# fujii-team/Henbun

Measured on AMD Instinct MI355X. Metric: elbo_samples_per_sec, higher is better.
Workload: dtype f32; 1 GPU; cfg2 SVGP ELBO step: 1-D UnitRBF, N=1e6, M=512 inducing, minibatch 8192 per GPU, diag Normal q(u), diagonal residual, Adam lr 1e-3; global_batch=8192, per_gpu_batch=8192, parallelism=dp1, N=1000000, M=512, dp_exchange=none, dp_ranks=1, contraction=native, tri_pack=False

## Files before the change

henbun_amd/csrc/chain.cuh:

```cuda
#ifndef HB_CHAIN_CUH
#define HB_CHAIN_CUH
#include "common.cuh"
#include "ew_prog.cuh"

enum { HB_CHAIN_PROG = 1, HB_CHAIN_ADAM = 2, HB_CHAIN_GLL = 3, HB_CHAIN_SGP_FINISH = 4, HB_CHAIN_GRAM_ELL = 5, HB_CHAIN_GLL_FOLD = 6 };
#define HB_CHAIN_MAX_JOBS 6
#define HB_CHAIN_PROG_MAX_N 4096
#define HB_CHAIN_FINISH_MAX_N 512
#define HB_CHAIN_GLL_MAX_N 4096
#define HB_CHAIN_ADAM_MAX_N 4096
#define HB_CHAIN_ELL_MAX_N 16384
#define HB_CHAIN_GLL_FOLD_MAX_N 4096

enum { HB_CHAIN_READ = 1, HB_CHAIN_WRITE = 2, HB_CHAIN_RW = 3 };

struct HbChainJob {
  int kind = 0, is64 = 0;
  const void* p[HB_PROG_MAX_IN + HB_PROG_MAX_OUT] = {};
  long l[8] = {};
  double d[8] = {};
  ProgArgs prog;
  int reduces = 0;
  long ext[HB_PROG_MAX_IN + HB_PROG_MAX_OUT] = {};
  unsigned char role[HB_PROG_MAX_IN + HB_PROG_MAX_OUT] = {};
  void span(int k, long bytes, int r) {
    ext[k] = p[k] != nullptr && bytes > 0 ? bytes : 0;
    role[k] = (unsigned char)r;
  }
};

bool hb_chain_recording();
int hb_chain_push(const HbChainJob& job, hipStream_t stream);
int hb_chain_flush(hipStream_t stream);

#endif
```

henbun_amd/csrc/chain_bodies.cuh:

```cuda
#ifndef HB_CHAIN_BODIES_CUH
#define HB_CHAIN_BODIES_CUH

#pragma clang fp contract(off)

__device__ __forceinline__ long hb_opaque_zero() {
  int z = 0;
  asm volatile("" : "+v"(z));
  return (long)z;
}

template <typename T>
struct HbAdamStatus {
  long tnow, fail0;
  T dpf;
  int w0;
};
template <typename T>
__device__ __forceinline__ void hb_adam_status_load(const long* t, const int* info, long n_info, const T* dpflag, const long* fail,
                                                    HbAdamStatus<T>& s) {
  const long z = hb_opaque_zero();
  const long* fp = fail != nullptr ? fail : t;
  const T* dp = dpflag != nullptr ? dpflag : reinterpret_cast<const T*>(t);
  const int* ip = n_info > 0 ? info + ((long)threadIdx.x < n_info ? (long)threadIdx.x : n_info - 1) : reinterpret_cast<const int*>(t);
  s.tnow = t[z];
// ... 263 lines not shown
  hb_gauss_fold_load<T, 1>(partial, nb, h);
  hb_gauss_fold_body<T, 1>(h, partial, nb, ll, dscale, dvar, smem, mir);
}

template <typename T>
__device__ __forceinline__ void sgp_finish_one(const T* __restrict__ part, int gy, long idx, T epsv, T* __restrict__ f,
                                               T* __restrict__ v, T* __restrict__ eps_out, long n, long P, int diagonal) {
  const long e = idx / n, j = idx - e * n;
  const T* pp = part + e * gy * 5 * n + j;
  T s = T(0);
  for (int y = 0; y < gy; ++y) s += pp[(long)y * 5 * n];
  const T vv = T(1) - s;
  v[idx] = vv;
  if (eps_out) eps_out[idx] = epsv;
  const T scale = diagonal ? hb_sqrt(hb_abs(vv)) * epsv : T(0);
  for (long p = 0; p < P; ++p) {
    T mean = T(0);
    for (int y = 0; y < gy; ++y) mean += pp[((long)y * 5 + 1 + p) * n];
    f[(e * P + p) * n + j] = mean + scale;
  }
}

template <typename T>
__device__ __forceinline__ void hb_sgp_finish_body(const T* __restrict__ part, int gy, const T* __restrict__ eps_in, uint64_t* rng,
                                                   long nlanes, T* __restrict__ eps_out, T* __restrict__ f, T* __restrict__ v,
                                                   long total, long n, long P, int diagonal, long t0, long nthreads) {
  const long npairs = (total + 1) / 2;
  if (rng) {
    const long nact = nlanes < npairs ? nlanes : npairs;
    for (long t = t0; t < nact; t += nthreads) {
      HbRng g = rng_load(rng, nlanes, t);
      for (long p = t; p < npairs; p += nlanes) {
        T z0, z1;
        g.normal2(z0, z1);
        sgp_finish_one<T>(part, gy, 2 * p, z0, f, v, eps_out, n, P, diagonal);
        if (2 * p + 1 < total) sgp_finish_one<T>(part, gy, 2 * p + 1, z1, f, v, eps_out, n, P, diagonal);
      }
      rng_store(rng, nlanes, t, g);
    }
  } else {
    for (long idx = t0; idx < total; idx += nthreads)
      sgp_finish_one<T>(part, gy, idx, eps_in ? eps_in[idx] : T(0), f, v, (eps_out != eps_in) ? eps_out : nullptr, n, P, diagonal);
  }
}

template <typename T, int D>
__device__ __forceinline__ void hb_gram_ell_load(const T* __restrict__ partial, long rows, long d, long dl, long c, T (&h)[D]) {
  const long cnt = dl == 1 ? rows * d : rows;
#pragma unroll
  for (int k = 0; k < D; ++k) {
    const long t = (long)threadIdx.x + (long)k * blockDim.x, tc = t < cnt ? t : cnt - 1;
    h[k] = dl == 1 ? partial[tc] : partial[tc * d + c];
  }
}
template <typename T, int D>
__device__ __forceinline__ void hb_gram_ell_body(const T (&h)[D], const T* __restrict__ partial, long rows, long d, long dl, long c,
                                                 T* __restrict__ ellbar, T* smem, T* mir = nullptr) {
  const long cnt = dl == 1 ? rows * d : rows;
  T acc = T(0);
#pragma unroll
  for (int k = 0; k < D; ++k)
    if ((long)threadIdx.x + (long)k * blockDim.x < cnt) acc += h[k];
  if (dl == 1) {
#pragma unroll 4
    for (long t = (long)threadIdx.x + (long)D * blockDim.x; t < cnt; t += blockDim.x) acc += partial[t];
  } else {
#pragma unroll 4
    for (long r = (long)threadIdx.x + (long)D * blockDim.x; r < cnt; r += blockDim.x) acc += partial[r * d + c];
  }
  acc = block_sum(acc, smem);
  if (threadIdx.x == 0) {
    ellbar[c] = acc;
    if (mir) mir[0] = acc;
  }
}
template <typename T>
__device__ __forceinline__ void hb_gram_ell_body(const T* __restrict__ partial, long rows, long d, long dl, long c,
                                                 T* __restrict__ ellbar, T* smem, T* mir = nullptr) {
  T h[1];
  hb_gram_ell_load<T, 1>(partial, rows, d, dl, c, h);
  hb_gram_ell_body<T, 1>(h, partial, rows, d, dl, c, ellbar, smem, mir);
}

template <typename T, int D>
__device__ __forceinline__ void hb_chain_win_load(const T* base, long n, T (&h)[D]) {
#pragma unroll
  for (int k = 0; k < D; ++k) {
    const long i = (long)threadIdx.x + (long)k * blockDim.x;
    h[k] = base[i < n ? i : hb_opaque_zero()];
  }
}
template <typename T, int D>
__device__ __forceinline__ void hb_chain_win_store(T* win, long n, const T (&h)[D]) {
#pragma unroll
  for (int k = 0; k < D; ++k) {
    const long i = (long)threadIdx.x + (long)k * blockDim.x;
    if (i < n) win[i] = h[k];
  }
}
template <typename T>
__device__ __forceinline__ void hb_chain_mirror(const T* p, T v, const T* base, long n, T* win) {
  const long ob = (long)p - (long)base;
  if (ob >= 0 && ob < n * (long)sizeof(T)) win[ob / (long)sizeof(T)] = v;
}
__device__ __forceinline__ void hb_chain_sync() { __syncthreads(); }

#pragma clang fp contract(fast)
#endif
```

henbun_amd/csrc/gram.hip:

```cpp
#include "common.cuh"
#include "../../include/henbun_hip.h"
#include "chain.cuh"
#include "gram_value.cuh"

template <typename T>
__global__ void __launch_bounds__(256) gram_fwd_kernel(int kind, const T* __restrict__ X, long sX,
                                                       const T* __restrict__ X2, long sX2, const T* __restrict__ ell,
                                                       long sEll, long dl, T* __restrict__ K, long B, long n, long n2,
                                                       long d, T diag_add) {
  const long total = B * n * n2;
  const long stride = (long)gridDim.x * blockDim.x;
  for (long t = (long)blockIdx.x * blockDim.x + threadIdx.x; t < total; t += stride) {
    const long b = t / (n * n2);
    const long rem = t - b * n * n2;
    const long i = rem / n2, j = rem - i * n2;
    const T kv = gram_value<T>(kind, X + b * sX + i * d, X2 + b * sX2 + j * d, ell + b * sEll, dl, d);
    K[t] = (i == j) ? kv + diag_add : kv;
  }
}

template <typename T>
static int gram_fwd(int kind, const T* X, long sX, const T* X2, long sX2, const T* ell, long sEll, long dl, T* K,
                    long B, long n, long n2, long d, double diag_add, hipStream_t stream) {
  HB_REQUIRE(kind >= HB_KERN_RBF && kind <= HB_KERN_SQDIST, "hb_gram_fwd: unknown kernel kind %d", kind);
// ... 95 lines not shown
template <typename T>
static int gram_bwd(int kind_flags, const T* X, long sX, const T* X2, long sX2, const T* ell, long sEll, long dl,
                    const T* Kbar, T* Xbar, T* X2bar, T* ellbar, long B, long n, long n2, long d, T* ws,
                    hipStream_t stream) {
  const int kind = kind_flags & ~HB_KERN_KBAR_SYMMETRIC;
  HB_REQUIRE(kind >= HB_KERN_RBF && kind <= HB_KERN_SQDIST, "hb_gram_bwd: unknown kernel kind %d", kind);
  HB_REQUIRE(B >= 0 && n >= 0 && n2 >= 0 && d >= 1, "hb_gram_bwd: bad extents");
  HB_REQUIRE(dl == 1 || dl == d, "hb_gram_bwd: lengthscales must have 1 or d entries");
  HB_REQUIRE(sEll == 0 || sEll == dl, "hb_gram_bwd: lengthscale batch stride must be 0 or dl");
  HB_REQUIRE(X && X2 && ell && Kbar, "hb_gram_bwd: NULL pointer");
  HB_REQUIRE(!ellbar || ws, "hb_gram_bwd: ellbar needs workspace");
  HB_REQUIRE(B <= 65535, "hb_gram_bwd: batch too large");
  if (B == 0) return 0;
  if (hb_chain_recording()) {
    const int crc = hb_chain_flush(stream);
    if (crc) return crc;
  }
  if (n == 0 || n2 == 0) {
    if (Xbar && n > 0) HB_HIP(hb_zero_async(Xbar, sizeof(T) * B * n * d, stream));
    if (X2bar && n2 > 0) HB_HIP(hb_zero_async(X2bar, sizeof(T) * B * n2 * d, stream));
    if (ellbar) HB_HIP(hb_zero_async(ellbar, sizeof(T) * dl * (sEll != 0 ? B : 1), stream));
    return 0;
  }
  const bool sym = Xbar && X2bar == Xbar;
  const bool kbar_sym = (kind_flags & HB_KERN_KBAR_SYMMETRIC) != 0;
  HB_REQUIRE(!kbar_sym || sym, "hb_gram_bwd: HB_KERN_KBAR_SYMMETRIC only applies to the one-pass form (X2 == X, X2bar == Xbar)");
  HB_REQUIRE(!sym || (X == X2 && sX == sX2 && n == n2), "hb_gram_bwd: Xbar == X2bar requires X2 == X");
  if (Xbar || ellbar) {
    hipLaunchKernelGGL(gram_bwd_side_kernel<T>, dim3(n, B), dim3(256), 0, stream, kind, sym ? (kbar_sym ? 3 : 2) : 0, X, sX, X2, sX2, ell, sEll,
                       dl, Kbar, Xbar, ellbar ? ws : (T*)nullptr, n, n2, d);
    HB_LAUNCH_CHECK();
    if (ellbar) {
      const long rows_ = sEll != 0 ? n : B * n, groups_ = sEll != 0 ? B : 1;
      if (hb_chain_recording() && rows_ * d * groups_ <= HB_CHAIN_ELL_MAX_N && groups_ * dl <= 16 && !(X2bar && !sym)) {
        HbChainJob j;
        j.kind = HB_CHAIN_GRAM_ELL;
        j.is64 = sizeof(T) == 8;
        j.p[0] = ws, j.p[1] = ellbar;
        j.l[0] = rows_, j.l[1] = d, j.l[2] = dl, j.l[3] = groups_;
        j.span(0, groups_ * rows_ * d * (long)sizeof(T), HB_CHAIN_READ), j.span(1, groups_ * dl * (long)sizeof(T), HB_CHAIN_WRITE);
        return hb_chain_push(j, stream);
      }
      if (sEll != 0)
        hipLaunchKernelGGL(gram_ell_finish_kernel<T>, dim3(dl, B), dim3(256), 0, stream, ws, n, d, dl, ellbar);
      else
        hipLaunchKernelGGL(gram_ell_finish_kernel<T>, dim3(dl, 1), dim3(256), 0, stream, ws, B * n, d, dl, ellbar);
      HB_LAUNCH_CHECK();
    }
  }
  if (X2bar && !sym) {
    hipLaunchKernelGGL(gram_bwd_side_kernel<T>, dim3(n2, B), dim3(256), 0, stream, kind, 1, X, sX, X2, sX2, ell, sEll,
                       dl, Kbar, X2bar, (T*)nullptr, n, n2, d);
    HB_LAUNCH_CHECK();
  }
  return 0;
}
template <typename T>
static int gram_ell_fold(const T* partial, long rows, long d, long dl, long groups, T* ellbar, hipStream_t stream) {
  HB_REQUIRE(partial && ellbar && rows >= 1 && d >= 1 && groups >= 1 && (dl == 1 || dl == d), "hb_gram_ell_fold: bad arguments");
  if (hb_chain_recording() && rows * d * groups <= HB_CHAIN_ELL_MAX_N && groups * dl <= 16) {
    HbChainJob j;
    j.kind = HB_CHAIN_GRAM_ELL;
    j.is64 = sizeof(T) == 8;
    j.p[0] = partial, j.p[1] = ellbar;
    j.l[0] = rows, j.l[1] = d, j.l[2] = dl, j.l[3] = groups;
    j.span(0, groups * rows * d * (long)sizeof(T), HB_CHAIN_READ), j.span(1, groups * dl * (long)sizeof(T), HB_CHAIN_WRITE);
    return hb_chain_push(j, stream);
  }
  if (hb_chain_recording()) {
    const int crc = hb_chain_flush(stream);
    if (crc) return crc;
  }
  hipLaunchKernelGGL(gram_ell_finish_kernel<T>, dim3(dl, groups), dim3(256), 0, stream, partial, rows, d, dl, ellbar);
  HB_LAUNCH_CHECK();
  return 0;
}
extern "C" int hb_gram_ell_fold_f32(const float* partial, long rows, long d, long dl, long groups, float* ellbar, void* stream) {
  return gram_ell_fold<float>(partial, rows, d, dl, groups, ellbar, (hipStream_t)stream);
}
extern "C" int hb_gram_ell_fold_f64(const double* partial, long rows, long d, long dl, long groups, double* ellbar, void* stream) {
  return gram_ell_fold<double>(partial, rows, d, dl, groups, ellbar, (hipStream_t)stream);
}

extern "C" int hb_gram_bwd_f32(int kind, const float* X, long sX, const float* X2, long sX2, const float* ell,
                               long sEll, long dl, const float* Kbar, float* Xbar, float* X2bar, float* ellbar,
                               long B, long n, long n2, long d, float* ws, void* stream) {
  return gram_bwd<float>(kind, X, sX, X2, sX2, ell, sEll, dl, Kbar, Xbar, X2bar, ellbar, B, n, n2, d, ws,
                         (hipStream_t)stream);
}
extern "C" int hb_gram_bwd_f64(int kind, const double* X, long sX, const double* X2, long sX2, const double* ell,
                               long sEll, long dl, const double* Kbar, double* Xbar, double* X2bar, double* ellbar,
                               long B, long n, long n2, long d, double* ws, void* stream) {
  return gram_bwd<double>(kind, X, sX, X2, sX2, ell, sEll, dl, Kbar, Xbar, X2bar, ellbar, B, n, n2, d, ws,
                          (hipStream_t)stream);
}
```

henbun_amd/csrc/jit.hip:

```cpp
#include "common.cuh"
#include "../../include/henbun_hip.h"
#include "ew_prog.cuh"
#include "chain.cuh"
#include <dlfcn.h>
#include <stdarg.h>
#include <stdio.h>
#include <string.h>
#include <hip/hiprtc.h>
#include <map>
#include <mutex>
#include <string>
#include <vector>
#include "_gen/ew_jit_prelude.inc"

namespace {

struct Rtc {
  bool ok = false;
  hiprtcResult (*create)(hiprtcProgram*, const char*, const char*, int, const char**, const char**) = nullptr;
  hiprtcResult (*compile)(hiprtcProgram, int, const char**) = nullptr;
  hiprtcResult (*log_size)(hiprtcProgram, size_t*) = nullptr;
  hiprtcResult (*log)(hiprtcProgram, char*) = nullptr;
  hiprtcResult (*code_size)(hiprtcProgram, size_t*) = nullptr;
  hiprtcResult (*code)(hiprtcProgram, char*) = nullptr;
// ... 368 lines not shown
            height[r] > 1 ? "q" : "0");
  }
  s += "  }\n}\n";
  if (source_out && source_cap > 0) snprintf(source_out, (size_t)source_cap, "%s", s.c_str() + (sizeof(HB_EW_JIT_PRELUDE) - 1));
  if (!handle_out) {
    std::vector<char> co;
    return compile_to_code(s, &co);
  }
  Compiled c;
  const int rc = compile_source(s, &c);
  if (rc) return rc;
  JitProgram* p = new JitProgram;
  p->colprog = true;
  p->is64 = sizeof(T) == 8;
  p->fn = c.fn;
  p->n = n;
  p->grid = (unsigned)hb_stream_grid(n, 256);
  for (int k = 0; k < nin; ++k) p->ptrs.push_back(const_cast<void*>(in[k]));
  for (int k = 0; k < nout; ++k) p->ptrs.push_back(out[k]);
  for (size_t k = 0; k < p->ptrs.size(); ++k) p->argv.push_back(&p->ptrs[k]);
  *handle_out = p;
  return 0;
}

}

extern "C" int hb_ewise_colprog_build_f32(int ninstr, const int* code, const double* params, int nin, const void* const* in,
                                          const long* istrides, int nout, void* const* out, const int* out_regs,
                                          const long* ostrides, long R, long n, void** handle_out, char* source_out,
                                          long source_cap) {
  return colprog_build<float>(ninstr, code, params, nin, in, istrides, nout, out, out_regs, ostrides, R, n, handle_out, source_out,
                              source_cap);
}
extern "C" int hb_ewise_colprog_build_f64(int ninstr, const int* code, const double* params, int nin, const void* const* in,
                                          const long* istrides, int nout, void* const* out, const int* out_regs,
                                          const long* ostrides, long R, long n, void** handle_out, char* source_out,
                                          long source_cap) {
  return colprog_build<double>(ninstr, code, params, nin, in, istrides, nout, out, out_regs, ostrides, R, n, handle_out, source_out,
                               source_cap);
}

extern "C" int hb_ewise_jit_available(void) { return rtc().ok ? 1 : 0; }

extern "C" int hb_ewise_jit_build_f32(int ninstr, const int* code, const double* params, int nin, const void* const* in,
                                      const long* istrides, int nout, void* const* out, const int* out_regs,
                                      const long* ostrides, int ndim, const long* shape, void** handle_out, long* n_out,
                                      int* reduces_out, char* source_out, long source_cap) {
  return jit_build<float>(ninstr, code, params, nin, in, istrides, nout, out, out_regs, ostrides, ndim, shape, handle_out,
                          n_out, reduces_out, source_out, source_cap);
}
extern "C" int hb_ewise_jit_build_f64(int ninstr, const int* code, const double* params, int nin, const void* const* in,
                                      const long* istrides, int nout, void* const* out, const int* out_regs,
                                      const long* ostrides, int ndim, const long* shape, void** handle_out, long* n_out,
                                      int* reduces_out, char* source_out, long source_cap) {
  return jit_build<double>(ninstr, code, params, nin, in, istrides, nout, out, out_regs, ostrides, ndim, shape, handle_out,
                           n_out, reduces_out, source_out, source_cap);
}

namespace {

struct ChainState {
  bool recording = false;
  std::vector<HbChainJob> jobs;
};
thread_local ChainState g_chain;

struct HbChainArgs {
  const void* p[64];
  long l[48];
  double d[16];
};

constexpr int CHAIN_NSTAMP = 16;
unsigned long long* g_chain_stamps = nullptr;
const void* chain_stamp_buffer() { return g_chain_stamps; }
static void chain_job_slots(const HbChainJob& j, int* p, int* l, int* d) {
  switch (j.kind) {
    case HB_CHAIN_PROG: *p = j.prog.nin + j.prog.nout, *l = 0, *d = 0; break;
    case HB_CHAIN_ADAM: *p = 8, *l = 3, *d = 5; break;
    case HB_CHAIN_GLL: *p = 9, *l = 1, *d = 1; break;
    case HB_CHAIN_GLL_FOLD: *p = 4, *l = 1, *d = 0; break;
    case HB_CHAIN_SGP_FINISH: *p = 6, *l = 6, *d = 0; break;
    case HB_CHAIN_GRAM_ELL: *p = 2, *l = 4, *d = 0; break;
    default: *p = 20, *l = 8, *d = 8; break;
  }
}

int chain_source_plain(const std::vector<HbChainJob>& jobs, std::string* out, HbChainArgs* args, int* np_out, int* nl_out, int* nd_out,
                       bool stamps) {
  const bool is64 = jobs[0].is64 != 0;
  std::string s;
  int np = 0, nl = 0, nd = 0;
  auto P = [&](const void* v) { HbChainArgs& a = *args; a.p[np] = v; return np++; };
  auto L = [&](long v) { HbChainArgs& a = *args; a.l[nl] = v; return nl++; };
  auto D = [&](double v) { HbChainArgs& a = *args; a.d[nd] = v; return nd++; };
  for (size_t q = 0; q < jobs.size(); ++q) {
    const HbChainJob& j = jobs[q];
    HB_REQUIRE((j.is64 != 0) == is64, "hb_chain: jobs of different element types in one chain");
    HB_REQUIRE(np + 20 <= 64 && nl + 8 <= 48 && nd + 8 <= 16, "hb_chain: argument block exhausted");
    if (q) s += "  __syncthreads();\n";
    s += "  {\n";
    if (j.kind == HB_CHAIN_PROG) {
      const ProgArgs& G = j.prog;
      for (int k = 0; k < G.nin; ++k) appendf(s, "  const T* in%d = (const T*)A.p[%d];\n", k, P(j.p[k]));
      for (int k = 0; k < G.nout; ++k) appendf(s, "  T* out%d = (T*)A.p[%d];\n", k, P(j.p[G.nin + k]));
      char loop[96];
      snprintf(loop, sizeof(loop), "for (long i = threadIdx.x; i < %ldL; i += 1024) {", G.n);
      emit_program(s, G, loop);
    } else if (j.kind == HB_CHAIN_ADAM) {
      const int p0 = P(j.p[0]); P(j.p[1]); P(j.p[2]); P(j.p[3]); P(j.p[4]); P(j.p[5]); P(j.p[6]); P(j.p[7]);
      const int l0 = L(j.l[0]); L(j.l[1]); L(j.l[2]);
      const int d0 = D(j.d[0]); D(j.d[1]); D(j.d[2]); D(j.d[3]); D(j.d[4]);
      appendf(s, "  hb_adam_body<T>((T*)A.p[%d], (const T*)A.p[%d], (T*)A.p[%d], (T*)A.p[%d], A.l[%d], A.d[%d], A.d[%d], A.d[%d], "
                 "A.d[%d], A.d[%d], (long*)A.p[%d], (int)A.l[%d], (const int*)A.p[%d], A.l[%d], (const T*)A.p[%d], (long*)A.p[%d], "
                 "(long)threadIdx.x, 1024L, true, true);\n",
              p0, p0 + 1, p0 + 2, p0 + 3, l0, d0, d0 + 1, d0 + 2, d0 + 3, d0 + 4, p0 + 4, l0 + 2, p0 + 5, l0 + 1, p0 + 6, p0 + 7);
    } else if (j.kind == HB_CHAIN_GLL) {
      const int p0 = P(j.p[0]); P(j.p[1]); P(j.p[2]); P(j.p[3]); P(j.p[4]); P(j.p[5]); P(j.p[6]); P(j.p[7]); P(j.p[8]);
      const int l0 = L(j.l[0]);
      const int d0 = D(j.d[0]);
      appendf(s, "  hb_gauss_ll_single_body<T>((const T*)A.p[%d], (const T*)A.p[%d], (const T*)A.p[%d], (const T*)A.p[%d], A.l[%d], "
                 "(T*)A.p[%d], (T*)A.p[%d], (T*)A.p[%d], (T*)A.p[%d], smem, (T*)A.p[%d], (T)A.d[%d]);\n",
              p0, p0 + 1, p0 + 2, p0 + 3, l0, p0 + 4, p0 + 5, p0 + 6, p0 + 7, p0 + 8, d0);
    } else if (j.kind == HB_CHAIN_GLL_FOLD) {
      const int p0 = P(j.p[0]); P(j.p[1]); P(j.p[2]); P(j.p[3]);
      const int l0 = L(j.l[0]);
      appendf(s, "  hb_gauss_fold_body<T>((const T*)A.p[%d], A.l[%d], (T*)A.p[%d], (T*)A.p[%d], (T*)A.p[%d], smem);\n", p0, l0, p0 + 1,
              p0 + 2, p0 + 3);
    } else if (j.kind == HB_CHAIN_SGP_FINISH) {
      const int p0 = P(j.p[0]); P(j.p[1]); P(j.p[2]); P(j.p[3]); P(j.p[4]); P(j.p[5]);
      const int l0 = L(j.l[0]); L(j.l[1]); L(j.l[2]); L(j.l[3]); L(j.l[4]); L(j.l[5]);
      appendf(s, "  hb_sgp_finish_body<T>((const T*)A.p[%d], (int)A.l[%d], (const T*)A.p[%d], (uint64_t*)A.p[%d], A.l[%d], (T*)A.p[%d], "
                 "(T*)A.p[%d], (T*)A.p[%d], A.l[%d], A.l[%d], A.l[%d], (int)A.l[%d], (long)threadIdx.x, 1024L);\n",
              p0, l0, p0 + 1, p0 + 2, l0 + 1, p0 + 3, p0 + 4, p0 + 5, l0 + 2, l0 + 3, l0 + 4, l0 + 5);
    } else if (j.kind == HB_CHAIN_GRAM_ELL) {
      const int p0 = P(j.p[0]); P(j.p[1]);
      const int l0 = L(j.l[0]); L(j.l[1]); L(j.l[2]); L(j.l[3]);
      appendf(s, "  for (long grp = 0; grp < A.l[%d]; ++grp)\n    for (long c = 0; c < A.l[%d]; ++c)\n"
                 "      hb_gram_ell_body<T>((const T*)A.p[%d] + grp * A.l[%d] * A.l[%d], A.l[%d], A.l[%d], A.l[%d], c, "
                 "(T*)A.p[%d] + grp * A.l[%d], smem);\n",
              l0 + 3, l0 + 2, p0, l0, l0 + 1, l0, l0 + 1, l0 + 2, p0 + 1, l0 + 2);
    } else {
      HB_REQUIRE(false, "hb_chain: unknown job kind %d", j.kind);
    }
    s += "  }\n";
    if (stamps) appendf(s, "  const unsigned long long hb_st%d = clock64();\n", (int)q + 2);
  }
  if (stamps) {
    HB_REQUIRE(np < 64, "hb_chain: no pointer slot left for the stamps");
    const int ps = P(chain_stamp_buffer());
    appendf(s, "  if (threadIdx.x == 0) {\n    unsigned long long* sb = (unsigned long long*)A.p[%d];\n    sb[0] = %dULL; sb[1] = hb_st0; sb[2] = hb_st0;\n", ps,
            (int)jobs.size() + 2);
    for (size_t q = 0; q < jobs.size(); ++q) appendf(s, "    sb[%d] = hb_st%d;\n", (int)q + 3, (int)q + 2);
    s += "  }\n";
  }
  s += "}\n";
  std::string h = HB_EW_JIT_PRELUDE;
  h += "\n#define HB_JIT_OPAQUE(x) asm volatile(\"\" : \"+v\"(x))";
  appendf(h, "\nstruct HbChainArgs { const void* p[%d]; long l[%d]; double d[%d]; };", np > 0 ? np : 1, nl > 0 ? nl : 1, nd > 0 ? nd : 1);
  appendf(h, "\ntypedef %s T;\nextern \"C\" __global__ void __launch_bounds__(1024) hb_jit_kernel(const HbChainArgs Ain) {\n",
          is64 ? "double" : "float");
  h += "  __shared__ T smem[16];\n  const HbChainArgs A = Ain;\n";
  if (stamps) h += "  const unsigned long long hb_st0 = clock64();\n";
  *out = h + s;
  *np_out = np, *nl_out = nl, *nd_out = nd;
  return 0;
}

enum { CH_PLAIN = 0, CH_EXT = 1, CH_SLOT = 2, CH_WIN = 3 };
constexpr long CHAIN_WIN_BYTES = 40960;
constexpr int CHAIN_MAX_WIN = 8, CHAIN_MAX_SLOT = 16;
constexpr int CHAIN_HOIST_REGS = 40;

struct ChainWin {
  int job, idx;
  int cap;
  std::string nexpr;
};
struct ChainMirror { int kind, id; };
struct ChainCls { int kind = CH_PLAIN, id = -1; };

struct ChainPlan {
  const std::vector<HbChainJob>& jobs;
  size_t esz;
  std::vector<int> pbase, lbase, dbase;
  std::vector<ChainWin> wins;
  int nslot = 0;
  long win_bytes = 0;
  std::vector<std::vector<std::vector<ChainMirror>>> mirrors;
  std::vector<std::vector<int>> slot_of;

  explicit ChainPlan(const std::vector<HbChainJob>& j) : jobs(j), esz(j[0].is64 ? 8 : 4) {
    int np = 0, nl = 0, nd = 0;
    for (const HbChainJob& q : jobs) {
      pbase.push_back(np), lbase.push_back(nl), dbase.push_back(nd);
      int a, b, c;
      chain_job_slots(q, &a, &b, &c);
      np += a, nl += b, nd += c;
    }
    mirrors.assign(jobs.size(), std::vector<std::vector<ChainMirror>>(HB_PROG_MAX_IN + HB_PROG_MAX_OUT));
    slot_of.assign(jobs.size(), std::vector<int>(HB_PROG_MAX_IN + HB_PROG_MAX_OUT, -1));
  }
  static bool overlap(const HbChainJob& a, int i, const HbChainJob& b, int k) {
    const char *a0 = (const char*)a.p[i], *b0 = (const char*)b.p[k];
    return a.ext[i] > 0 && b.ext[k] > 0 && a0 < b0 + b.ext[k] && b0 < a0 + a.ext[i];
  }
  int capability(int j, int k) const {
    const HbChainJob& J = jobs[j];
    switch (J.kind) {
      case HB_CHAIN_PROG: return k >= J.prog.nin ? 2 : 0;
      case HB_CHAIN_ADAM: return k == 0 ? 2 : 0;
      case HB_CHAIN_GLL: return k >= 5 && k <= 7 ? 1 : 0;
      case HB_CHAIN_GLL_FOLD: return k >= 1 && k <= 3 ? 1 : 0;
      case HB_CHAIN_GRAM_ELL: return k == 1 && J.ext[1] == (long)esz ? 1 : 0;
      default: return 0;
    }
  }
  int slot(int j, int k) {
    if (slot_of[j][k] >= 0) return slot_of[j][k];
    const int kind = jobs[j].kind;
    const bool triple = kind == HB_CHAIN_GLL || kind == HB_CHAIN_GLL_FOLD;
    const int first = kind == HB_CHAIN_GLL ? 5 : kind == HB_CHAIN_GLL_FOLD ? 1 : k, count = triple ? 3 : 1;
    if (nslot + count > CHAIN_MAX_SLOT) return -1;
    for (int c = 0; c < count; ++c) slot_of[j][first + c] = nslot + c;
    nslot += count;
    return slot_of[j][k];
  }
  bool external(int q, int k) const {
    for (int j = 0; j < q; ++j)
      for (int o = 0; o < HB_PROG_MAX_IN + HB_PROG_MAX_OUT; ++o)
        if ((jobs[j].role[o] & HB_CHAIN_WRITE) && overlap(jobs[q], k, jobs[j], o)) return false;
    return true;
  }
  ChainCls classify(int q, int k, long n, const std::string& nexpr) {
    ChainCls c;
    const HbChainJob& Q = jobs[q];
    if (Q.ext[k] <= 0) return c;
    std::vector<std::pair<int, int>> prod;
    for (int j = 0; j < q; ++j)
      for (int o = 0; o < HB_PROG_MAX_IN + HB_PROG_MAX_OUT; ++o)
        if ((jobs[j].role[o] & HB_CHAIN_WRITE) && overlap(Q, k, jobs[j], o)) prod.push_back({j, o});
    if (prod.empty()) {
      c.kind = CH_EXT;
      return c;
    }
    if (prod.size() == 1 && n == 1) {
      const int j = prod[0].first, o = prod[0].second;
      if (jobs[j].p[o] == Q.p[k] && jobs[j].ext[o] == (long)esz && capability(j, o) >= 1) {
        const int sl = slot(j, o);
        if (sl < 0) return c;
        mirrors[j][o].push_back({CH_SLOT, sl});
        c.kind = CH_SLOT, c.id = sl;
        return c;
      }
    }
    int cap = 1;
    while (cap < n) cap *= 2;
    if ((int)wins.size() >= CHAIN_MAX_WIN || n < 1 || win_bytes + (long)cap * (long)esz > CHAIN_WIN_BYTES) return c;
    for (const auto& jo : prod) {
      const long off = (const char*)jobs[jo.first].p[jo.second] - (const char*)Q.p[k];
      if (capability(jo.first, jo.second) != 2 || off % (long)esz != 0) return c;
    }
    const int w = (int)wins.size();
    wins.push_back({q, k, cap, nexpr});
    win_bytes += (long)cap * (long)esz;
    for (const auto& jo : prod) mirrors[jo.first][jo.second].push_back({CH_WIN, w});
    c.kind = CH_WIN, c.id = w;
    return c;
  }
  std::string mirror_text(int j, int k) const {
    std::string t;
    for (const ChainMirror& m : mirrors[j][k]) {
      if (m.kind == CH_SLOT) {
        appendf(t, "hb_slot[%d] = %%V; ", m.id);
      } else {
        const ChainWin& W = wins[m.id];
        appendf(t, "hb_chain_mirror<T>(%%P, %%V, (const T*)A.p[%d], %s, hb_win%d); ", pbase[W.job] + W.idx, W.nexpr.c_str(), m.id);
      }
    }
    return t;
  }
  std::string mir_arg(int j, int k) const {
    char b[48];
    if (slot_of[j][k] >= 0)
      snprintf(b, sizeof(b), "hb_slot + %d", slot_of[j][k]);
    else
      snprintf(b, sizeof(b), "(T*)nullptr");
    return b;
  }
};

int chain_source_hoist(const std::vector<HbChainJob>& jobs, std::string* out, HbChainArgs* args, int* np_out, int* nl_out, int* nd_out,
                       bool stamps) {
  const bool is64 = jobs[0].is64 != 0;
  const int NQ = (int)jobs.size();
  int np = 0, nl = 0, nd = 0;
  auto P = [&](const void* v) { HbChainArgs& a = *args; a.p[np] = v; return np++; };
  auto L = [&](long v) { HbChainArgs& a = *args; a.l[nl] = v; return nl++; };
  auto D = [&](double v) { HbChainArgs& a = *args; a.d[nd] = v; return nd++; };
  ChainPlan plan(jobs);
  struct JobCls {
    ChainCls in[HB_PROG_MAX_IN];
    bool hoist = false;
    ChainCls g;
    bool tmv_ext = false, st_ext = false, part_ext = false;
    int depth = 1;
  };
  std::vector<JobCls> cls(NQ);
  for (int q = 0; q < NQ; ++q) {
    const HbChainJob& j = jobs[q];
    HB_REQUIRE((j.is64 != 0) == is64, "hb_chain: jobs of different element types in one chain");
    JobCls& c = cls[q];
    if (j.kind == HB_CHAIN_PROG) {
      const ProgArgs& G = j.prog;
      c.hoist = G.n >= 1 && G.n <= 1024;
      for (int k = 0; k < G.nin && c.hoist; ++k) {
        long n = 1;
        for (int d = 0; d < G.ndim; ++d) n += G.istr[k][d] * (long)(G.shape[d] - 1);
        char b[32];
        snprintf(b, sizeof(b), "%ldL", n);
        c.in[k] = plan.classify(q, k, n, b);
      }
    } else if (j.kind == HB_CHAIN_ADAM) {
      c.depth = (int)((j.l[0] + 1023) / 1024);
      c.tmv_ext = plan.external(q, 0) && plan.external(q, 2) && plan.external(q, 3);
      c.st_ext = plan.external(q, 4) && plan.external(q, 5) && plan.external(q, 6) && plan.external(q, 7);
      char b[32];
      snprintf(b, sizeof(b), "A.l[%d]", plan.lbase[q]);
      c.g = plan.classify(q, 1, j.l[0], b);
    } else if (j.kind == HB_CHAIN_GLL_FOLD) {
      c.part_ext = plan.external(q, 0);
      c.depth = (int)((j.l[0] + 1023) / 1024);
    } else if (j.kind == HB_CHAIN_GRAM_ELL) {
      c.part_ext = plan.external(q, 0);
      c.depth = (int)(((j.l[2] == 1 ? j.l[0] * j.l[1] : j.l[0]) + 1023) / 1024);
    }
    if (c.depth < 1) c.depth = 1;
  }
  int held = 0;
  for (const ChainWin& W : plan.wins) held += (W.cap > 1024 ? W.cap / 1024 : 1) * (is64 ? 2 : 1);
  auto fits = [&](int values) {
    const int regs = values * (is64 ? 2 : 1);
    if (held + regs > CHAIN_HOIST_REGS) return false;
    held += regs;
    return true;
  };
  for (int pass = 0; pass < 2; ++pass) {
    for (int q = 0; q < NQ; ++q) {
      const HbChainJob& j = jobs[q];
      JobCls& c = cls[q];
      if ((j.kind == HB_CHAIN_ADAM) != (pass == 0)) continue;
      if (j.kind == HB_CHAIN_ADAM) {
        if (c.tmv_ext && !fits(3 * c.depth)) c.tmv_ext = false;
        if (c.g.kind == CH_EXT && !fits(c.depth)) c.g.kind = CH_PLAIN;
      } else if (j.kind == HB_CHAIN_GLL_FOLD) {
        if (c.part_ext && !fits(3 * c.depth)) c.part_ext = false;
      } else if (j.kind == HB_CHAIN_GRAM_ELL) {
        if (c.part_ext && !fits(c.depth)) c.part_ext = false;
      } else if (j.kind == HB_CHAIN_PROG) {
        for (int k = 0; k < j.prog.nin; ++k)
          if (c.in[k].kind == CH_EXT && !fits(1)) c.in[k].kind = CH_PLAIN;
      }
    }
  }
  std::string top, s;
  for (size_t w = 0; w < plan.wins.size(); ++w) {
    const ChainWin& W = plan.wins[w];
    const int dw = W.cap > 1024 ? W.cap / 1024 : 1;
    appendf(top, "  T hb_wf%d[%d]; hb_chain_win_load<T, %d>((const T*)A.p[%d], %s, hb_wf%d);\n", (int)w, dw, dw, plan.pbase[W.job] + W.idx,
            W.nexpr.c_str(), (int)w);
  }
  for (int q = 0; q < NQ; ++q) {
    const HbChainJob& j = jobs[q];
    const JobCls& c = cls[q];
    HB_REQUIRE(np + 20 <= 64 && nl + 8 <= 48 && nd + 8 <= 16, "hb_chain: argument block exhausted");
    HB_REQUIRE(np == plan.pbase[q] && nl == plan.lbase[q] && nd == plan.dbase[q], "hb_chain: argument slots out of step");
    if (q) s += "  __syncthreads();\n";
    s += "  {\n";
    if (j.kind == HB_CHAIN_PROG) {
      const ProgArgs& G = j.prog;
      ProgHooks hooks;
      for (int k = 0; k < G.nin; ++k) appendf(s, "  const T* in%d = (const T*)A.p[%d];\n", k, P(j.p[k]));
      for (int k = 0; k < G.nout; ++k) appendf(s, "  T* out%d = (T*)A.p[%d];\n", k, P(j.p[G.nin + k]));
      bool any_ext = false;
      for (int k = 0; k < G.nin; ++k) any_ext = any_ext || c.in[k].kind == CH_EXT;
      if (any_ext) {
        appendf(top, "  const long h%di = (long)threadIdx.x < %ldL ? (long)threadIdx.x : 0L;\n  long h%drem = h%di;\n", q, G.n, q, q);
        for (int d = G.ndim - 1; d >= 0; --d) {
          if (d == 0)
            appendf(top, "  const long h%dx%d = h%drem;\n", q, d, q);
          else
            appendf(top, "  const long h%dx%d = h%drem %% %dL; h%drem /= %dL;\n", q, d, q, G.shape[d], q, G.shape[d]);
        }
      }
      for (int k = 0; k < G.nin; ++k) {
        char b[256];
        if (c.in[k].kind == CH_EXT) {
          bool uniform = true;
          for (int d = 0; d < G.ndim; ++d) uniform = uniform && G.istr[k][d] == 0;
          appendf(top, "  const T h%d_%d = ((const T*)A.p[%d])[%s", q, k, plan.pbase[q] + k, uniform ? "hb_opaque_zero()" : "0");
          for (int d = 0; d < G.ndim; ++d)
            if (G.istr[k][d] != 0) appendf(top, " + h%dx%d * %ldL", q, d, G.istr[k][d]);
          top += "];\n";
          snprintf(b, sizeof(b), "h%d_%d", q, k);
          hooks.in_expr[k] = b;
        } else if (c.in[k].kind == CH_SLOT) {
          snprintf(b, sizeof(b), "hb_slot[%d]", c.in[k].id);
          hooks.in_expr[k] = b;
        } else if (c.in[k].kind == CH_WIN) {
          std::string e;
          appendf(e, "hb_win%d[0", c.in[k].id);
          for (int d = 0; d < G.ndim; ++d)
            if (G.istr[k][d] != 0) appendf(e, " + x%d * %ldL", d, G.istr[k][d]);
          hooks.in_expr[k] = e + "]";
        }
      }
      for (int k = 0; k < G.nout; ++k) hooks.out_extra[k] = plan.mirror_text(q, G.nin + k);
      char loop[96];
      snprintf(loop, sizeof(loop), "for (long i = threadIdx.x; i < %ldL; i += 1024) {", G.n);
      emit_program(s, G, loop, &hooks);
    } else if (j.kind == HB_CHAIN_ADAM) {
      const int p0 = P(j.p[0]); P(j.p[1]); P(j.p[2]); P(j.p[3]); P(j.p[4]); P(j.p[5]); P(j.p[6]); P(j.p[7]);
      const int l0 = L(j.l[0]); L(j.l[1]); L(j.l[2]);
      const int d0 = D(j.d[0]); D(j.d[1]); D(j.d[2]); D(j.d[3]); D(j.d[4]);
      std::string status, tmv, lr, gload;
      appendf(top, "  HbAdamOps<T, %d> h%do; HbAdamStatus<T> h%ds;\n", c.depth, q, q);
      appendf(status, "  hb_adam_status_load<T>((const long*)A.p[%d], (const int*)A.p[%d], A.l[%d], (const T*)A.p[%d], (const long*)A.p[%d], h%ds);\n",
              p0 + 4, p0 + 5, l0 + 1, p0 + 6, p0 + 7, q);
      appendf(tmv, "  hb_adam_load_tmv<T, %d>((const T*)A.p[%d], (const T*)A.p[%d], (const T*)A.p[%d], A.l[%d], (long)threadIdx.x, 1024L, h%do);\n",
              c.depth, p0, p0 + 2, p0 + 3, l0, q);
      appendf(lr, "  const T h%dlr = hb_adam_lr<T>(A.d[%d], A.d[%d], A.d[%d], h%ds.tnow);\n", q, d0, d0 + 1, d0 + 2, q);
      if (c.g.kind == CH_WIN)
        appendf(gload, "  hb_adam_load_g<T, %d>(hb_win%d, A.l[%d], (long)threadIdx.x, 1024L, h%do);\n", c.depth, c.g.id, l0, q);
      else
        appendf(gload, "  hb_adam_load_g<T, %d>((const T*)A.p[%d], A.l[%d], (long)threadIdx.x, 1024L, h%do);\n", c.depth, p0 + 1, l0, q);
      (c.st_ext ? top : s) += status;
      (c.tmv_ext ? top : s) += tmv;
      (c.g.kind == CH_EXT ? top : s) += gload;
      const int lr_slot = c.st_ext && q > 0 && plan.nslot < CHAIN_MAX_SLOT ? plan.nslot++ : -1;
      if (lr_slot >= 0) {
        appendf(top, "  if ((threadIdx.x >> 6) == 15) {\n  %s    if ((threadIdx.x & 63) == 0) hb_slot[%d] = h%dlr;\n  }\n", lr.c_str(), lr_slot, q);
        appendf(s, "  const T h%dlr = hb_slot[%d];\n", q, lr_slot);
      } else {
        (c.st_ext ? top : s) += lr;
      }
      std::string fn = "HbNoMirror()";
      const std::string mt = plan.mirror_text(q, 0);
      if (!mt.empty()) fn = "[&](const T* hp, T hv) { " + hook_text(mt, "hp", "hv") + "}";
      appendf(s, "  if (!hb_adam_status_blocked<T>(h%ds, (const long*)A.p[%d], (const int*)A.p[%d], A.l[%d], (const T*)A.p[%d], (long*)A.p[%d], true)) {\n",
              q, p0 + 4, p0 + 5, l0 + 1, p0 + 6, p0 + 7);
      appendf(s, "    hb_adam_body<T>((T*)A.p[%d], (const T*)A.p[%d], (T*)A.p[%d], (T*)A.p[%d], A.l[%d], h%dlr, A.d[%d], A.d[%d], A.d[%d], "
                 "A.d[%d], (long)threadIdx.x, 1024L, h%do, %s);\n",
              p0, p0 + 1, p0 + 2, p0 + 3, l0, q, d0 + 1, d0 + 2, d0 + 3, d0 + 4, q, fn.c_str());
      appendf(s, "    if (A.l[%d]) hb_adam_tick((long*)A.p[%d], h%ds.tnow);\n  }\n", l0 + 2, p0 + 4, q);
    } else if (j.kind == HB_CHAIN_GLL) {
      const int p0 = P(j.p[0]); P(j.p[1]); P(j.p[2]); P(j.p[3]); P(j.p[4]); P(j.p[5]); P(j.p[6]); P(j.p[7]); P(j.p[8]);
      const int l0 = L(j.l[0]);
      const int d0 = D(j.d[0]);
      appendf(s, "  hb_gauss_ll_single_body<T>((const T*)A.p[%d], (const T*)A.p[%d], (const T*)A.p[%d], (const T*)A.p[%d], A.l[%d], "
                 "(T*)A.p[%d], (T*)A.p[%d], (T*)A.p[%d], (T*)A.p[%d], smem, (T*)A.p[%d], (T)A.d[%d], %s);\n",
              p0, p0 + 1, p0 + 2, p0 + 3, l0, p0 + 4, p0 + 5, p0 + 6, p0 + 7, p0 + 8, d0, plan.mir_arg(q, 5).c_str());
    } else if (j.kind == HB_CHAIN_GLL_FOLD) {
      const int p0 = P(j.p[0]); P(j.p[1]); P(j.p[2]); P(j.p[3]);
      const int l0 = L(j.l[0]);
      if (c.part_ext) {
        appendf(top, "  T h%dp[%d]; hb_gauss_fold_load<T, %d>((const T*)A.p[%d], A.l[%d], h%dp);\n", q, 3 * c.depth, c.depth, p0, l0, q);
        appendf(s, "  hb_gauss_fold_body<T, %d>(h%dp, (const T*)A.p[%d], A.l[%d], (T*)A.p[%d], (T*)A.p[%d], (T*)A.p[%d], smem, %s);\n", c.depth, q,
                p0, l0, p0 + 1, p0 + 2, p0 + 3, plan.mir_arg(q, 1).c_str());
      } else {
        appendf(s, "  hb_gauss_fold_body<T>((const T*)A.p[%d], A.l[%d], (T*)A.p[%d], (T*)A.p[%d], (T*)A.p[%d], smem, %s);\n", p0, l0, p0 + 1,
                p0 + 2, p0 + 3, plan.mir_arg(q, 1).c_str());
      }
    } else if (j.kind == HB_CHAIN_SGP_FINISH) {
      const int p0 = P(j.p[0]); P(j.p[1]); P(j.p[2]); P(j.p[3]); P(j.p[4]); P(j.p[5]);
      const int l0 = L(j.l[0]); L(j.l[1]); L(j.l[2]); L(j.l[3]); L(j.l[4]); L(j.l[5]);
      appendf(s, "  hb_sgp_finish_body<T>((const T*)A.p[%d], (int)A.l[%d], (const T*)A.p[%d], (uint64_t*)A.p[%d], A.l[%d], (T*)A.p[%d], "
                 "(T*)A.p[%d], (T*)A.p[%d], A.l[%d], A.l[%d], A.l[%d], (int)A.l[%d], (long)threadIdx.x, 1024L);\n",
              p0, l0, p0 + 1, p0 + 2, l0 + 1, p0 + 3, p0 + 4, p0 + 5, l0 + 2, l0 + 3, l0 + 4, l0 + 5);
    } else if (j.kind == HB_CHAIN_GRAM_ELL) {
      const int p0 = P(j.p[0]); P(j.p[1]);
      const int l0 = L(j.l[0]); L(j.l[1]); L(j.l[2]); L(j.l[3]);
      const std::string mir = plan.mir_arg(q, 1);
      if (c.part_ext) {
        appendf(top, "  T h%dp[%d]; hb_gram_ell_load<T, %d>((const T*)A.p[%d], A.l[%d], A.l[%d], A.l[%d], 0L, h%dp);\n", q, c.depth, c.depth, p0,
                l0, l0 + 1, l0 + 2, q);
        appendf(s, "  hb_gram_ell_body<T, %d>(h%dp, (const T*)A.p[%d], A.l[%d], A.l[%d], A.l[%d], 0L, (T*)A.p[%d], smem, %s);\n", c.depth, q, p0,
                l0, l0 + 1, l0 + 2, p0 + 1, mir.c_str());
      }
      appendf(s, "  for (long grp = 0; grp < A.l[%d]; ++grp)\n    for (long c = %s; c < A.l[%d]; ++c)\n"
                 "      hb_gram_ell_body<T>((const T*)A.p[%d] + grp * A.l[%d] * A.l[%d], A.l[%d], A.l[%d], A.l[%d], c, "
                 "(T*)A.p[%d] + grp * A.l[%d], smem, %s);\n",
              l0 + 3, c.part_ext ? "(grp == 0 ? 1L : 0L)" : "0L", l0 + 2, p0, l0, l0 + 1, l0, l0 + 1, l0 + 2, p0 + 1, l0 + 2,
              c.part_ext ? "(T*)nullptr" : mir.c_str());
    } else {
      HB_REQUIRE(false, "hb_chain: unknown job kind %d", j.kind);
    }
    s += "  }\n";
    if (stamps) appendf(s, "  const unsigned long long hb_st%d = clock64();\n", q + 2);
  }
  if (stamps) {
    HB_REQUIRE(np < 64, "hb_chain: no pointer slot left for the stamps");
    const int ps = P(chain_stamp_buffer());
    appendf(s, "  if (threadIdx.x == 0) {\n    unsigned long long* sb = (unsigned long long*)A.p[%d];\n    sb[0] = %dULL; sb[1] = hb_st0; sb[2] = hb_st1;\n", ps, NQ + 2);
    for (int q = 0; q < NQ; ++q) appendf(s, "    sb[%d] = hb_st%d;\n", q + 3, q + 2);
    s += "  }\n";
  }
  s += "}\n";
  std::string h = HB_EW_JIT_PRELUDE;
  h += "\n#define HB_JIT_OPAQUE(x) asm volatile(\"\" : \"+v\"(x))";
  appendf(h, "\nstruct HbChainArgs { const void* p[%d]; long l[%d]; double d[%d]; };", np > 0 ? np : 1, nl > 0 ? nl : 1, nd > 0 ? nd : 1);
  appendf(h, "\ntypedef %s T;\nextern \"C\" __global__ void __launch_bounds__(1024) hb_jit_kernel(const HbChainArgs Ain) {\n",
          is64 ? "double" : "float");
  h += "  __shared__ T smem[16];\n";
  if (plan.nslot) appendf(h, "  __shared__ T hb_slot[%d];\n", plan.nslot);
  for (size_t w = 0; w < plan.wins.size(); ++w) appendf(h, "  __shared__ T hb_win%d[%d];\n", (int)w, plan.wins[w].cap);
  h += "  const HbChainArgs A = Ain;\n";
  if (stamps) h += "  const unsigned long long hb_st0 = clock64();\n";
  h += top;
  for (size_t w = 0; w < plan.wins.size(); ++w) {
    const ChainWin& W = plan.wins[w];
    appendf(h, "  hb_chain_win_store<T, %d>(hb_win%d, %s, hb_wf%d);\n", W.cap > 1024 ? W.cap / 1024 : 1, (int)w, W.nexpr.c_str(), (int)w);
  }
  if (!plan.wins.empty()) h += "  hb_chain_sync();\n";
  if (stamps) h += "  const unsigned long long hb_st1 = clock64();\n";
  *out = h + s;
  *np_out = np, *nl_out = nl, *nd_out = nd;
  return 0;
}

int chain_source(const std::vector<HbChainJob>& jobs, std::string* out, HbChainArgs* args, int* np_out, int* nl_out, int* nd_out) {
  const bool stamps = hb_debug_get("chain_stamps", 0) != 0;
  bool plain = hb_debug_get("chain_hoist", 1) == 0;
  for (const HbChainJob& j : jobs) {
    if (j.kind != HB_CHAIN_PROG) continue;
    for (int d = 0; d < j.prog.ndim; ++d) {
      for (int k = 0; k < j.prog.nin; ++k) plain = plain || j.prog.istr[k][d] < 0;
      for (int k = 0; k < j.prog.nout; ++k) plain = plain || j.prog.ostr[k][d] < 0;
    }
  }
  bool has_adam = false;
  for (const HbChainJob& j : jobs) has_adam = has_adam || j.kind == HB_CHAIN_ADAM;
  plain = plain || !has_adam;
  if (plain) return chain_source_plain(jobs, out, args, np_out, nl_out, nd_out, stamps);
  return chain_source_hoist(jobs, out, args, np_out, nl_out, nd_out, stamps);
}

}

bool hb_chain_recording() { return g_chain.recording; }

int hb_chain_flush(hipStream_t stream) {
  if (g_chain.jobs.empty()) return 0;
  std::vector<HbChainJob> jobs;
  jobs.swap(g_chain.jobs);
  std::string src;
  HbChainArgs args = {};
  int np = 0, nl = 0, nd = 0;
  HB_REQUIRE(hb_debug_get("chain_stamps", 0) == 0 || g_chain_stamps != nullptr,
             "hb_chain: chain_stamps is set but hb_chain_stamps has not been called (it allocates the stamp buffer)");
  int rc = chain_source(jobs, &src, &args, &np, &nl, &nd);
  if (rc) return rc;
  Compiled c;
  rc = compile_source(src, &c);
  if (rc) return rc;
  unsigned char packed[sizeof(HbChainArgs)];
  const size_t bp = sizeof(void*) * (size_t)(np > 0 ? np : 1), bl = sizeof(long) * (size_t)(nl > 0 ? nl : 1),
               bd = sizeof(double) * (size_t)(nd > 0 ? nd : 1);
  memcpy(packed, args.p, bp);
  memcpy(packed + bp, args.l, bl);
  memcpy(packed + bp + bl, args.d, bd);
  size_t size = bp + bl + bd;
  void* config[] = {HIP_LAUNCH_PARAM_BUFFER_POINTER, packed, HIP_LAUNCH_PARAM_BUFFER_SIZE, &size, HIP_LAUNCH_PARAM_END};
  HB_HIP(hipModuleLaunchKernel(c.fn, 1, 1, 1, 1024, 1, 1, 0, stream, nullptr, config));
  return 0;
}

// ... 113 lines not shown
```

henbun_amd/csrc/linalg.hip:

```cpp
#include "common.cuh"
#include "sgp_strip.cuh"
#include "side_jobs.cuh"
#include "gemm_tile.cuh"
#include "../../include/henbun_hip.h"

template <typename T>
struct MmArgs {
  const T* A;
  const T* B;
  T* C;
  long M, N, K, lda, ldb, ldc, sA, sB, sC, batch;
  T alpha, beta;
  const T* bias;
  long sBias;
  int act, flags, S, tile;
  int to_ws;
  int bfast;
  T* ws;
  T* colsum;
  T* colsum_ws;
};

template <typename T>
__device__ __forceinline__ T apply_act(int act, T v) {
  switch (act) {
    case HB_ACT_SIGMOID: return hb_sigmoid(v);
    case HB_ACT_RELU: return v > T(0) ? v : T(0);
    case HB_ACT_TANH: return hb_tanh(v);
    default: return v;
  }
}

template <typename T>
__device__ __forceinline__ T act_grad(int act, T y) {
  switch (act) {
    case HB_ACT_SIGMOID: return y * (T(1) - y);
    case HB_ACT_RELU: return y > T(0) ? T(1) : T(0);
    case HB_ACT_TANH: return T(1) - y * y;
    default: return T(1);
  }
}

template <typename T, bool TA, bool TB, int BT>
struct MmBK {
  static constexpr int value = 16;
};

template <typename T, bool TA, bool TB, bool FAST, int BT>
__global__ void __launch_bounds__(256) matmul_kernel(MmArgs<T> a) {
  typedef TileGemm<T, BT, BT, MmBK<T, TA, TB, BT>::value, 2, 2> G;
  __shared__ __attribute__((aligned(16))) T lds[G::LDS_ELEMS];
  const int M = (int)a.M, N = (int)a.N, K = (int)a.K;
  const int lda = (int)a.lda, ldb = (int)a.ldb;
  const int tiles_n = (N + BT - 1) / BT;
  int tile, s;
  long b;
  if (a.bfast) {
    b = blockIdx.x % a.batch;
    const int rest = (int)(blockIdx.x / a.batch);
    const int ntile = tiles_n * ((M + BT - 1) / BT);
    s = rest / ntile;
    tile = rest - s * ntile;
  } else {
    tile = blockIdx.x / a.S;
    s = blockIdx.x - tile * a.S;
    b = blockIdx.y;
  }
  const int row0 = (tile / tiles_n) * BT;
  const int col0 = (tile % tiles_n) * BT;
  if ((a.flags & (HB_MM_LOWER_OUT | HB_MM_TRIL_OUT | HB_MM_PHI_OUT | HB_MM_SYMLOW_OUT)) && col0 > row0 + BT - 1) {
    if ((a.flags & (HB_MM_TRIL_OUT | HB_MM_PHI_OUT)) && !a.to_ws) {
      T* Cb = a.C + b * a.sC;
      for (int idx = threadIdx.x; idx < BT * BT; idx += 256) {
        const int r = row0 + idx / BT, c = col0 + idx % BT;
        if (r < M && c < N) Cb[(long)r * a.ldc + c] = T(0);
      }
    }
    return;
  }
  int kchunk = (K + a.S - 1) / a.S;
  kchunk = ((kchunk + G::BK - 1) / G::BK) * G::BK;
  const int kbeg = s * kchunk;
  int kend = kbeg + kchunk;
  if (kend > K) kend = K;
  const T* Ab = a.A + b * a.sA;
  const T* Bb = a.B + b * a.sB;
// ... 111 lines not shown
__global__ void __launch_bounds__(256) matmul_splitk_finish_kernel(MmArgs<T> a) {
  const long total = a.batch * a.M * a.N;
  const long stride = (long)gridDim.x * blockDim.x;
  if ((a.flags & HB_MM_COLSUM_B) && a.colsum) {
    const int sl = threadIdx.x & 15;
    for (long cb = blockIdx.x; cb * 16 < a.N; cb += gridDim.x) {
      const long c = cb * 16 + (threadIdx.x >> 4);
      const long cc = c < a.N ? c : a.N - 1;
      T v[8];
#pragma unroll
      for (int q = 0; q < 8; ++q) {
        const int s = sl + 16 * q;
        v[q] = s < a.S ? a.colsum_ws[(long)s * a.N + cc] : T(0);
      }
      T acc = ((v[0] + v[1]) + (v[2] + v[3])) + ((v[4] + v[5]) + (v[6] + v[7]));
#pragma unroll
      for (int off = 8; off > 0; off >>= 1) acc += __shfl_xor(acc, off, 16);
      if (sl == 0 && c < a.N) a.colsum[c] = acc;
    }
  }
  for (long t = (long)blockIdx.x * blockDim.x + threadIdx.x; t < total; t += stride) {
    const long b = t / (a.M * a.N);
    const long rem = t - b * a.M * a.N;
    const long r = rem / a.N, c = rem - r * a.N;
    T* cp = a.C + b * a.sC + r * a.ldc + c;
    if ((a.flags & (HB_MM_TRIL_OUT | HB_MM_PHI_OUT)) && c > r) {
      cp[0] = T(0);
      continue;
    }
    if ((a.flags & HB_MM_LOWER_OUT) && (c / a.tile) * a.tile > (r / a.tile) * a.tile + a.tile - 1) continue;
    auto slab_sum = [&](long at) -> T {
      T acc0 = T(0), acc1 = T(0), acc2 = T(0), acc3 = T(0);
      int s = 0;
      for (; s + 16 <= a.S; s += 16) {
        T v[16];
#pragma unroll
        for (int q = 0; q < 16; ++q) v[q] = a.ws[(long)(s + q) * total + at];
#pragma unroll
        for (int q = 0; q < 16; q += 4) acc0 += v[q], acc1 += v[q + 1], acc2 += v[q + 2], acc3 += v[q + 3];
      }
      for (; s + 4 <= a.S; s += 4) {
        const T v0 = a.ws[(long)s * total + at], v1 = a.ws[(long)(s + 1) * total + at];
        const T v2 = a.ws[(long)(s + 2) * total + at], v3 = a.ws[(long)(s + 3) * total + at];
        acc0 += v0, acc1 += v1, acc2 += v2, acc3 += v3;
      }
      for (; s < a.S; ++s) acc0 += a.ws[(long)s * total + at];
      return (acc0 + acc1) + (acc2 + acc3);
    };
    if (a.flags & HB_MM_SYMLOW_OUT) {
      cp[0] = T(0.5) * slab_sum(c > r ? b * a.M * a.N + c * a.N + r : t);
      continue;
    }
    T acc = slab_sum(t);
    if (a.flags & HB_MM_SYM_OUT) {
      const long tt = b * a.M * a.N + c * a.N + r;
      const T acc2 = slab_sum(tt);
      cp[0] = T(0.5) * (acc + acc2);
      continue;
    }
    if (a.flags & HB_MM_ACTGRAD) {
      cp[0] = acc * act_grad<T>(a.act, a.bias[b * a.sBias + r * a.N + c]);
      continue;
    }
    if (a.bias) acc += a.bias[b * a.sBias + c];
    acc = apply_act<T>(a.act, acc);
    if (a.beta != T(0)) acc += a.beta * cp[0];
    if ((a.flags & HB_MM_PHI_OUT) && c == r) acc *= T(0.5);
    cp[0] = acc;
  }
}

#define WGK_LD 33
struct MmGramVjp {
  const float* X = nullptr;
  long sX = 0;
  const float* ell = nullptr;
  long sEll = 0, dl = 1, d = 1;
  float* Xbar = nullptr;
  float* ell_partial = nullptr;
  float* part = nullptr;
  unsigned* counters = nullptr;
};
#define HB_MMG_MAXD 4
template <bool TA, bool TB, bool SYM>
__global__ void __launch_bounds__(256) matmul_wgk_kernel(MmArgs<float> a, int nown, HbSideJobs side, MmGramVjp gv) {
  if ((int)blockIdx.x >= nown) {
    if (blockIdx.y == 0) hb_side_run(side, (int)blockIdx.x - nown);
    return;
  }
  typedef float V4 __attribute__((ext_vector_type(4)));
  typedef Mma<float> MM;
  __shared__ float red[SYM ? 8 : 4][32][WGK_LD];
  const int M = (int)a.M, N = (int)a.N, K = (int)a.K;
  const int lda = (int)a.lda, ldb = (int)a.ldb;
  const int tiles_n = N / 32;
  const long b = blockIdx.y;
  int ti, tj;
  if (SYM) {
    int t = blockIdx.x;
    ti = (int)((sqrtf(8.f * (float)t + 1.f) - 1.f) * 0.5f);
    while (ti * (ti + 1) / 2 > t) --ti;
    while ((ti + 1) * (ti + 2) / 2 <= t) ++ti;
    tj = t - ti * (ti + 1) / 2;
  } else {
    ti = blockIdx.x / tiles_n;
    tj = blockIdx.x - ti * tiles_n;
  }
  const int row0 = ti * 32, col0 = tj * 32;
  const int tid = threadIdx.x, lane = tid & 63, w = __builtin_amdgcn_readfirstlane(tid >> 6), li = lane & 31, h = lane >> 5;
  float* Cb = a.C + b * a.sC;
  const bool lower_only = (a.flags & (HB_MM_LOWER_OUT | HB_MM_TRIL_OUT | HB_MM_PHI_OUT | HB_MM_SYMLOW_OUT)) != 0;
  if (!SYM && lower_only && col0 > row0 + 31) {
    if (a.flags & (HB_MM_TRIL_OUT | HB_MM_PHI_OUT)) {
      for (int idx = tid; idx < 1024; idx += 256) Cb[(long)(row0 + (idx >> 5)) * a.ldc + col0 + (idx & 31)] = 0.f;
    }
    return;
  }
  const float* __restrict__ Ab = a.A + b * a.sA;
  const float* __restrict__ Bb = a.B + b * a.sB;
  const int Kw = K / 4, kbeg = w * Kw, nch = Kw / 32;
  typename MM::Acc acc, acc2;
#pragma unroll
  for (int r = 0; r < 16; ++r) acc[r] = 0.f, acc2[r] = 0.f;

  constexpr int CH = SYM ? 2 : 4;
  struct Frag {
    float a[CH][16], b[CH][16], a2[SYM ? CH : 1][16], b2[SYM ? CH : 1][16];
  };
  auto load_side = [&](float (&f)[16], const float* __restrict__ base, int ld, bool kmajor, int idx0, int k0) {
    if (kmajor) {
#pragma unroll
      for (int j = 0; j < 16; ++j) f[j] = base[(long)(k0 + 16 * h + j) * ld + idx0 + li];
    } else {
      const float* p = base + (long)(idx0 + li) * ld + k0 + 16 * h;
#pragma unroll
      for (int v = 0; v < 4; ++v) {
        const V4 q = *reinterpret_cast<const V4*>(p + 4 * v);
#pragma unroll
        for (int s2 = 0; s2 < 4; ++s2) f[4 * v + s2] = q[s2];
      }
    }
  };
  auto load = [&](Frag& f, int c0) {
    if (c0 >= nch) return;
#pragma unroll
    for (int q = 0; q < CH; ++q) {
      const int cc = c0 + q < nch ? c0 + q : nch - 1;
      const int k0 = kbeg + 32 * cc;
      load_side(f.a[q], Ab, lda, TA, row0, k0);
      load_side(f.b[q], Bb, ldb, !TB, col0, k0);
      if (SYM) {
        load_side(f.a2[q], Ab, lda, TA, col0, k0);
        load_side(f.b2[q], Bb, ldb, !TB, row0, k0);
      }
    }
  };
  auto compute = [&](const Frag& f, int c0) {
#pragma unroll
    for (int q = 0; q < CH; ++q) {
      if (c0 + q >= nch) break;
#pragma unroll
      for (int j = 0; j < 16; ++j) {
        acc = MM::mma(f.a[q][j], f.b[q][j], acc);
        if (SYM) acc2 = MM::mma(f.a2[q][j], f.b2[q][j], acc2);
      }
    }
  };
  {
    Frag fa, fb;
    load(fa, 0);
#pragma nounroll
    for (int c = 0; c < nch; c += 2 * CH) {
      load(fb, c + CH);
      __builtin_amdgcn_sched_barrier(0);
      compute(fa, c);
      __builtin_amdgcn_sched_barrier(0);
      load(fa, c + 2 * CH);
      __builtin_amdgcn_sched_barrier(0);
      compute(fb, c + CH);
      __builtin_amdgcn_sched_barrier(0);
    }
  }
#pragma unroll
  for (int r = 0; r < 16; ++r) {
    red[w][MM::acc_row(lane, r)][li] = acc[r];
    if (SYM) red[4 + w][MM::acc_row(lane, r)][li] = acc2[r];
  }
  __syncthreads();
  const float* biasb = a.bias ? a.bias + b * a.sBias : nullptr;
  float gval[4];
#pragma unroll
  for (int e = 0; e < 4; ++e) {
    const int idx = tid + 256 * e, r = idx >> 5, c = idx & 31;
    float v = ((red[0][r][c] + red[1][r][c]) + (red[2][r][c] + red[3][r][c])) * a.alpha;
    gval[e] = v;
    const long gr = row0 + r, gcn = col0 + c;
    if (SYM) {
      const float vm = ((red[4][c][r] + red[5][c][r]) + (red[6][c][r] + red[7][c][r])) * a.alpha;
      const float sy = 0.5f * (v + vm);
      Cb[gr * a.ldc + gcn] = sy;
      continue;
    }
    if (a.flags & HB_MM_SYMLOW_OUT) {
      const int rr = (ti == tj && c > r) ? c : r, cc = (ti == tj && c > r) ? r : c;
      Cb[gr * a.ldc + gcn] = 0.5f * a.alpha * ((red[0][rr][cc] + red[1][rr][cc]) + (red[2][rr][cc] + red[3][rr][cc]));
      continue;
    }
    if (biasb) v += biasb[gcn];
    v = apply_act<float>(a.act, v);
    if (a.beta != 0.f) v += a.beta * Cb[gr * a.ldc + gcn];
    if ((a.flags & (HB_MM_TRIL_OUT | HB_MM_PHI_OUT)) && gcn > gr) v = 0.f;
    if ((a.flags & HB_MM_PHI_OUT) && gcn == gr) v *= 0.5f;
    Cb[gr * a.ldc + gcn] = v;
  }
  if (!SYM && gv.X) {
    const int d = (int)gv.d, c = tid & 31;
    const float* Xb = gv.X + b * gv.sX;
    const float* eb = gv.ell + b * gv.sEll;
    float il[HB_MMG_MAXD], xj[HB_MMG_MAXD];
#pragma unroll
    for (int k = 0; k < HB_MMG_MAXD; ++k) {
      il[k] = k < d ? 1.f / eb[gv.dl == 1 ? 0 : k] : 0.f;
      xj[k] = k < d ? Xb[(long)(col0 + c) * d + k] : 0.f;
    }
    const int tiles_m = M / 32;
    float* pt = gv.part + ((((long)b * tiles_m + ti) * tiles_n + tj) * 32) * 2 * d;
#pragma unroll
    for (int e = 0; e < 4; ++e) {
      const int r = (tid >> 5) + 8 * e;
      float dm[HB_MMG_MAXD], r2 = 0.f;
#pragma unroll
      for (int k = 0; k < HB_MMG_MAXD; ++k) {
        dm[k] = k < d ? (Xb[(long)(row0 + r) * d + k] * il[k] - xj[k] * il[k]) : 0.f;
        r2 += dm[k] * dm[k];
      }
      const float km = hb_exp(-0.5f * r2), kb = gval[e];
      const float em = kb * km, gm = (kb + kb) * km;
#pragma unroll
      for (int k = 0; k < HB_MMG_MAXD; ++k) {
        if (k < d) {
          float ga = (-dm[k] * gm) * il[k], la = (dm[k] * dm[k] * em) * il[k];
#pragma unroll
          for (int off = 16; off > 0; off >>= 1) {
            ga += __shfl_xor(ga, off, 32);
            la += __shfl_xor(la, off, 32);
          }
          if (c == 0) {
            __hip_atomic_store(pt + r * 2 * d + k, ga, __ATOMIC_RELAXED, __HIP_MEMORY_SCOPE_AGENT);
            __hip_atomic_store(pt + r * 2 * d + d + k, la, __ATOMIC_RELAXED, __HIP_MEMORY_SCOPE_AGENT);
          }
        }
      }
    }
    asm volatile("s_waitcnt vmcnt(0)" ::: "memory");
    __shared__ unsigned s_lastg;
    __syncthreads();
    if (tid == 0) {
      const unsigned old = __hip_atomic_fetch_add(gv.counters + b * tiles_m + ti, 1u, __ATOMIC_RELAXED, __HIP_MEMORY_SCOPE_AGENT);
      s_lastg = old == (unsigned)tiles_n - 1u ? 1u : 0u;
    }
    __syncthreads();
    if (s_lastg) {
      const float* p0 = gv.part + (((long)b * tiles_m + ti) * tiles_n) * 32 * 2 * d;
      for (int idx = tid; idx < 32 * 2 * d; idx += 256) {
        float sum = 0.f;
        for (int t = 0; t < tiles_n; ++t) sum += __hip_atomic_load(const_cast<float*>(p0) + (long)t * 32 * 2 * d + idx, __ATOMIC_RELAXED, __HIP_MEMORY_SCOPE_AGENT);
        const int r = idx / (2 * d), q = idx - r * 2 * d;
        if (q < d)
          gv.Xbar[((long)b * M + row0 + r) * d + q] = sum;
        else
          gv.ell_partial[((long)b * M + row0 + r) * d + q - d] = sum;
      }
      if (tid == 0) __hip_atomic_store(gv.counters + b * tiles_m + ti, 0u, __ATOMIC_RELAXED, __HIP_MEMORY_SCOPE_AGENT);
    }
  }
  if (!SYM && (a.flags & HB_MM_SYMLOW_OUT) && ti != tj) {
#pragma unroll
    for (int e = 0; e < 4; ++e) {
      const int idx = tid + 256 * e, r = idx >> 5, c = idx & 31;
      Cb[(long)(col0 + r) * a.ldc + row0 + c] = 0.5f * a.alpha * ((red[0][c][r] + red[1][c][r]) + (red[2][c][r] + red[3][c][r]));
    }
  }
  if (SYM && ti != tj) {
#pragma unroll
    for (int e = 0; e < 4; ++e) {
      const int idx = tid + 256 * e, r = idx >> 5, c = idx & 31;
      const float v = ((red[0][c][r] + red[1][c][r]) + (red[2][c][r] + red[3][c][r])) * a.alpha;
      const float vm = ((red[4][r][c] + red[5][r][c]) + (red[6][r][c] + red[7][r][c])) * a.alpha;
      Cb[(long)(col0 + r) * a.ldc + row0 + c] = 0.5f * (v + vm);
    }
  }
}

extern "C" int hb_matmul_wgk_shape(long M, long N, long K, long batch) {
  if (M % 32 || N % 32 || K % 128 || K < 128 || K > 4096) return 0;
  return (M / 32) * (N / 32) * batch <= 1024 && batch <= 65535 ? 1 : 0;
}
template <typename T>
static bool matmul_wgk_ok(const MmArgs<T>&, long, long, long, long, int, bool) { return false; }
template <>
bool matmul_wgk_ok<float>(const MmArgs<float>& a, long M, long N, long K, long batch, int flags, bool aligned) {
  const bool off = hb_debug_get("mm_no_wgk", 0) != 0;
  if (off || !aligned || !hb_matmul_wgk_shape(M, N, K, batch)) return false;
  if (flags & HB_MM_ACTGRAD) return false;
  return !((flags & HB_MM_SYM_OUT) && M != N);
}
template <typename T>
static int matmul_wgk_launch(const MmArgs<T>&, int, int, hipStream_t) { return -1; }
int matmul_wgk_launch_g(const MmArgs<float>& a, int transA, int transB, hipStream_t stream, const MmGramVjp& gv);
template <>
int matmul_wgk_launch<float>(const MmArgs<float>& a, int transA, int transB, hipStream_t stream) { return matmul_wgk_launch_g(a, transA, transB, stream, MmGramVjp()); }
int matmul_wgk_launch_g(const MmArgs<float>& a, int transA, int transB, hipStream_t stream, const MmGramVjp& gv) {
  const bool sym = (a.flags & HB_MM_SYM_OUT) != 0;
  const long nt = a.M / 32;
  const int nown = (int)(sym ? nt * (nt + 1) / 2 : (a.M / 32) * (a.N / 32));
  const HbSideJobs sj = hb_side_take();
  dim3 grid((unsigned)(nown + sj.total), (unsigned)a.batch, 1);
#define HB_WGK(TA_, TB_)                                                                                   \
  do {                                                                                                     \
    if (sym)                                                                                               \
      hipLaunchKernelGGL((matmul_wgk_kernel<TA_, TB_, true>), grid, dim3(256), 0, stream, a, nown, sj, gv);    \
    else                                                                                                   \
      hipLaunchKernelGGL((matmul_wgk_kernel<TA_, TB_, false>), grid, dim3(256), 0, stream, a, nown, sj, gv);   \
  } while (0)
  if (!transA && !transB)
    HB_WGK(false, false);
  else if (!transA && transB)
    HB_WGK(false, true);
  else if (transA && !transB)
    HB_WGK(true, false);
  else
    HB_WGK(true, true);
#undef HB_WGK
  HB_LAUNCH_CHECK();
  return 0;
}

#define RS_LDS_FLOATS 18432
template <bool TB, int NT, int WC, int G, int NW>
__global__ void __launch_bounds__(64 * NW, NW == 8 ? 4 : 2) matmul_rows_kernel(MmArgs<float> a) {
  typedef float V4 __attribute__((ext_vector_type(4)));
  typedef Mma<float> MM;
  __shared__ __attribute__((aligned(16))) float Ws[RS_LDS_FLOATS];
  const int M = (int)a.M, N = (int)a.N, K = (int)a.K;
  const int lda = (int)a.lda, ldb = (int)a.ldb, ldc = (int)a.ldc;
  const int KLD = K + 4;
  const int tid = threadIdx.x, lane = tid & 63, w = __builtin_amdgcn_readfirstlane(tid >> 6), li = lane & 31, h = lane >> 5;
  constexpr int NP = 32 * NT * WC, ROWS = 32 * (NW / WC), NTHR = 64 * NW;
  const int wr = w / WC, wc = w % WC;
  {
    const int kq = K >> 2;
    if (TB) {
      for (int idx = tid; idx < NP * kq; idx += NTHR) {
        const int c = idx / kq, k4 = idx - c * kq;
        V4 v = {0.f, 0.f, 0.f, 0.f};
        if (c < N) v = *reinterpret_cast<const V4*>(a.B + (long)c * ldb + 4 * k4);
        *reinterpret_cast<V4*>(&Ws[c * KLD + 4 * k4]) = v;
      }
    } else {
      for (int idx = tid; idx < NP * kq; idx += NTHR) {
        const int k4 = idx / NP, c = idx - k4 * NP;
        V4 v = {0.f, 0.f, 0.f, 0.f};
        if (c < N) {
#pragma unroll
          for (int i = 0; i < 4; ++i) v[i] = a.B[(long)(4 * k4 + i) * ldb + c];
        }
        *reinterpret_cast<V4*>(&Ws[c * KLD + 4 * k4]) = v;
      }
    }
  }
  const int cbase = 32 * NT * wc;
  float breg[NT];
#pragma unroll
  for (int t = 0; t < NT; ++t) {
    const int c = cbase + 32 * t + li;
    breg[t] = (a.bias && !(a.flags & HB_MM_ACTGRAD) && c < N) ? a.bias[c] : 0.f;
  }
  __syncthreads();
  const int nchunk = K / (2 * G);
  const int ntile = (M + ROWS - 1) / ROWS;
  for (int tile = blockIdx.x; tile < ntile; tile += gridDim.x) {
    const int r0 = tile * ROWS + 32 * wr;
    if (r0 >= M || cbase >= N) continue;
    const int arow = r0 + li < M ? r0 + li : M - 1;
    const float* __restrict__ ap = a.A + (long)arow * lda + G * h;
    typename MM::Acc acc[NT];
#pragma unroll
    for (int t = 0; t < NT; ++t)
#pragma unroll
      for (int r = 0; r < 16; ++r) acc[t][r] = 0.f;
    auto load = [&](V4 (&f)[G / 4], int c) {
      const int cc = c < nchunk ? c : nchunk - 1;
#pragma unroll
      for (int v = 0; v < G / 4; ++v) f[v] = *reinterpret_cast<const V4*>(ap + 2 * G * cc + 4 * v);
    };
    auto compute = [&](const V4 (&f)[G / 4], int c) {
      if (c >= nchunk) return;
#pragma unroll
      for (int t = 0; t < NT; ++t) {
        const float* wp = &Ws[(cbase + 32 * t + li) * KLD + 2 * G * c + G * h];
        V4 bv[G / 4];
#pragma unroll
        for (int v = 0; v < G / 4; ++v) bv[v] = *reinterpret_cast<const V4*>(wp + 4 * v);
#pragma unroll
// ... 533 lines not shown
  return 0;
}

extern "C" int hb_matmul_colsum_f32(const float* A, const float* B, float* C, float* colsum, long M, long N, long K, long lda,
                                    long ldb, long ldc, float* ws, long ws_elems, void* stream) {
  HB_REQUIRE(colsum && ldb == N, "hb_matmul_colsum: colsum is NULL or B is not contiguous (ldb != N)");
  return matmul_launch<float>(A, B, C, 1, M, N, K, lda, ldb, ldc, 0, 0, 0, 1, 0, 1.0, 0.0, nullptr, 0, HB_ACT_NONE, 0, ws,
                              ws_elems, (hipStream_t)stream, colsum);
}
extern "C" int hb_matmul_colsum_f64(const double* A, const double* B, double* C, double* colsum, long M, long N, long K,
                                    long lda, long ldb, long ldc, double* ws, long ws_elems, void* stream) {
  HB_REQUIRE(colsum && ldb == N, "hb_matmul_colsum: colsum is NULL or B is not contiguous (ldb != N)");
  return matmul_launch<double>(A, B, C, 1, M, N, K, lda, ldb, ldc, 0, 0, 0, 1, 0, 1.0, 0.0, nullptr, 0, HB_ACT_NONE, 0, ws,
                               ws_elems, (hipStream_t)stream, colsum);
}

extern "C" int hb_matmul_f32(const float* A, const float* B, float* C, long batch, long M, long N, long K, long lda,
                             long ldb, long ldc, long sA, long sB, long sC, int transA, int transB, double alpha,
                             double beta, const float* bias, long sBias, int act, int flags, float* ws, long ws_elems,
                             void* stream) {
  return matmul_launch<float>(A, B, C, batch, M, N, K, lda, ldb, ldc, sA, sB, sC, transA, transB, alpha, beta, bias,
                              sBias, act, flags, ws, ws_elems, (hipStream_t)stream);
}
template <typename T>
static int matmul_form_query(long batch, long M, long N, long K, long lda, long ldb, long ldc, long sA, long sB, int transA,
                             int transB, double beta, int flags, int a_aligned, int b_aligned, long ws_elems, int colsum,
                             int* S, int* vec, int* finish, int* bfast, int* colsum_fused) {
  MmArgs<T> a = {};
  a.A = (const T*)(uintptr_t)(a_aligned ? 256 : 256 + sizeof(T));
  a.B = (const T*)(uintptr_t)(b_aligned ? 256 : 256 + sizeof(T));
  a.M = M, a.N = N, a.K = K, a.lda = lda, a.ldb = ldb, a.ldc = ldc, a.sA = sA, a.sB = sB, a.batch = batch;
  a.beta = (T)beta, a.flags = flags;
  if (colsum) ws_elems -= 128 * N;
  if (ws_elems < 0) ws_elems = 0;
  if (matmul_reject_flags(batch, M, N, beta, flags, ws_elems)) return -1;
  const MmForm f = matmul_decide<T>(a, transA, transB, ws_elems, colsum != 0);
  const bool tile = f.form == HB_MM_FORM_TILE64 || f.form == HB_MM_FORM_TILE128;
  if (tile && !matmul_grid_ok(f, batch, M, N)) return -1;
  if (S) *S = tile ? f.S : 1;
  if (vec) *vec = tile ? f.vec : 0;
  if (finish) *finish = tile ? f.to_ws : 0;
  if (bfast) *bfast = tile ? f.bfast : 0;
  if (colsum_fused) *colsum_fused = tile ? f.colsum_fused : 0;
  return f.form;
}
extern "C" int hb_matmul_form(int elem_bytes, long batch, long M, long N, long K, long lda, long ldb, long ldc, long sA, long sB,
                              int transA, int transB, double beta, int flags, int a_aligned, int b_aligned, long ws_elems,
                              int colsum, int* S, int* vec, int* finish, int* bfast, int* colsum_fused) {
  if ((elem_bytes != 4 && elem_bytes != 8) || batch < 1 || M < 1 || N < 1 ||
      matmul_reject_extents(batch, M, N, K, lda, ldb, ldc, transA, transB) || (colsum && ws_elems <= 128 * N))
    return -1;
  if (colsum && (batch != 1 || !transA || transB || ldb != N || flags != 0 || beta != 0.0)) return -1;
  if (elem_bytes == 4)
    return matmul_form_query<float>(batch, M, N, K, lda, ldb, ldc, sA, sB, transA, transB, beta, flags, a_aligned, b_aligned,
                                    ws_elems, colsum, S, vec, finish, bfast, colsum_fused);
  return matmul_form_query<double>(batch, M, N, K, lda, ldb, ldc, sA, sB, transA, transB, beta, flags, a_aligned, b_aligned,
                                   ws_elems, colsum, S, vec, finish, bfast, colsum_fused);
}

extern "C" int hb_matmul_gram_vjp_ok(long M, long K, long batch, long d) {
  MmArgs<float> t = {};
  if (hb_debug_get("mm_no_gram_vjp", 0) != 0 || d < 1 || d > HB_MMG_MAXD) return 0;
  return matmul_wgk_ok<float>(t, M, M, K, batch, 0, true) ? 1 : 0;
}
extern "C" long hb_matmul_gram_vjp_ws_elems(long batch, long M, long d) { return batch * (M / 32) * (M / 32) * 32 * 2 * d; }
extern "C" int hb_matmul_gram_vjp_f32(const float* A, const float* B, float* C, long batch, long M, long K, long lda, long ldb,
                                      long ldc, long sA, long sB, long sC, int transA, int transB, const float* X, long sX,
                                      const float* ell, long sEll, long dl, long d, float* Xbar, float* ell_partial,
                                      float* part, unsigned* counters, void* stream) {
  HB_REQUIRE(A && B && C && X && ell && Xbar && ell_partial && part && counters, "hb_matmul_gram_vjp: NULL pointer");
  HB_REQUIRE(hb_matmul_gram_vjp_ok(M, K, batch, d), "hb_matmul_gram_vjp: shape outside the in-workgroup split-K form (hb_matmul_gram_vjp_ok)");
  HB_REQUIRE(dl == 1 || dl == d, "hb_matmul_gram_vjp: lengthscales must have 1 or d entries");
  const bool aligned = ((uintptr_t)A % 16 == 0) && ((uintptr_t)B % 16 == 0) && ((uintptr_t)C % 16 == 0) && lda % 4 == 0 && ldb % 4 == 0 && ldc % 4 == 0;
  HB_REQUIRE(aligned, "hb_matmul_gram_vjp: operands must be 16-byte aligned with leading dimensions %% 4 == 0");
  HB_REQUIRE(lda >= (transA ? M : K) && ldb >= (transB ? K : M) && ldc >= M, "hb_matmul_gram_vjp: leading dimension too small");
  MmArgs<float> a = {};
  a.A = A, a.B = B, a.C = C;
  a.M = M, a.N = M, a.K = K, a.lda = lda, a.ldb = ldb, a.ldc = ldc, a.sA = sA, a.sB = sB, a.sC = sC, a.batch = batch;
  a.alpha = 1.f, a.beta = 0.f, a.act = HB_ACT_NONE, a.flags = 0;
  MmGramVjp gv;
  gv.X = X, gv.sX = sX, gv.ell = ell, gv.sEll = sEll, gv.dl = dl, gv.d = d;
  gv.Xbar = Xbar, gv.ell_partial = ell_partial, gv.part = part, gv.counters = counters;
  return matmul_wgk_launch_g(a, transA, transB, (hipStream_t)stream, gv);
}

static inline bool matmul_gauss_shape(long n, long K, long N, int& G, int& KC) {
  if (hb_debug_get("mm_no_gauss_head", 0) != 0) return false;
  if (n < 2048 || N <= 32 || N > 256 || n * N >= 2147483647L) return false;
  MmArgs<float> t = {};
  t.N = N, t.K = K;
  return matmul_rowsreg_ok(t, G, KC);
}
extern "C" long hb_matmul_gauss_units(long n, long K, long N) {
  int G, KC;
  if (!matmul_gauss_shape(n, K, N, G, KC)) return 0;
  return 4 * matmul_rowsreg_wgs(n, N, KC);
}
extern "C" int hb_matmul_gauss_f32(const float* A, long lda, const float* B, long ldb, const float* bias, const float* y,
                                   const float* scale, const float* var, double post, float* dmu, float* fbar, float* part,
                                   long units, long n, long K, long N, void* stream) {
  int G, KC;
  HB_REQUIRE(A && B && y && var && dmu && part, "hb_matmul_gauss: NULL pointer");
  HB_REQUIRE(matmul_gauss_shape(n, K, N, G, KC) && units == 4 * matmul_rowsreg_wgs(n, N, KC),
             "hb_matmul_gauss: units must be hb_matmul_gauss_units(n, K, N) > 0 (n = %ld, K = %ld, N = %ld)", n, K, N);
  HB_REQUIRE((uintptr_t)A % 16 == 0 && lda % 4 == 0 && lda >= K && ldb >= N, "hb_matmul_gauss: A must be 16-byte aligned with lda %% 4 == 0");
  MmArgs<float> a = {};
  a.A = A, a.B = B, a.C = dmu, a.bias = bias;
  a.M = n, a.N = N, a.K = K, a.lda = lda, a.ldb = ldb, a.ldc = N;
  a.batch = 1, a.alpha = 1.f, a.beta = 0.f, a.act = HB_ACT_NONE, a.flags = 0;
  MmHead hd;
  hd.y = y, hd.scale = scale, hd.var = var, hd.post = (float)post, hd.fbar = fbar, hd.part = part, hd.units = units;
  return matmul_rowsreg_launch(a, 0, G, KC, (hipStream_t)stream, &hd);
}

extern "C" int hb_matmul_f64(const double* A, const double* B, double* C, long batch, long M, long N, long K,
                             long lda, long ldb, long ldc, long sA, long sB, long sC, int transA, int transB,
                             double alpha, double beta, const double* bias, long sBias, int act, int flags, double* ws,
                             long ws_elems, void* stream) {
  return matmul_launch<double>(A, B, C, batch, M, N, K, lda, ldb, ldc, sA, sB, sC, transA, transB, alpha, beta, bias,
                               sBias, act, flags, ws, ws_elems, (hipStream_t)stream);
}


template <typename T>
__global__ void __launch_bounds__(256) tril_inplace_kernel(T* __restrict__ L, T* __restrict__ W, T* __restrict__ Wf, int bf16x3,
                                                           long B, long M) {
  const int Mi = (int)M;
  const long mm = M * M, total = B * mm;
  const long stride = (long)gridDim.x * blockDim.x;
  const int nT = Mi / 32;
  for (long t = (long)blockIdx.x * blockDim.x + threadIdx.x; t < total; t += stride) {
    const long b = t / mm;
    const int rem = (int)(t - b * mm);
    const int i = rem / Mi, j = rem - i * Mi;
    if (j > i) {
      L[t] = T(0);
      if (W) W[t] = T(0);
    }
    if (Wf) {
      const T* Wb = W + b * mm;
      {
        const int s = rem & 3, lane = (rem >> 2) & 63, v = (rem >> 8) & 3, blk = rem >> 10;
        const int Q = blk % nT, tt = blk / nT, li = lane & 31, h = lane >> 5;
        const int r = 32 * tt + li, k = 32 * Q + 16 * h + 4 * v + s;
        Wf[t] = k <= r ? Wb[(long)r * Mi + k] : T(0);
        Wf[total + t] = r <= k ? Wb[(long)k * Mi + r] : T(0);
      }
      if (bf16x3) {
        const int jj = rem & 7, lane = (rem >> 3) & 63, q = (rem >> 9) & 1, blk = rem >> 10;
        const int Q = blk % nT, tt = blk / nT, li = lane & 31, h = lane >> 5;
        const int r = 32 * tt + li, k = 32 * Q + 16 * q + 8 * h + jj;
        __bf16* W3 = reinterpret_cast<__bf16*>(Wf + 2 * total);
        const float x = k <= r ? (float)Wb[(long)r * Mi + k] : 0.f;
        const float xt = r <= k ? (float)Wb[(long)k * Mi + r] : 0.f;
        __bf16 a0, a1, a2;
        hb_split_bf16x3(x, a0, a1, a2);
        W3[t] = a0, W3[total + t] = a1, W3[2 * total + t] = a2;
        hb_split_bf16x3(xt, a0, a1, a2);
        W3[3 * total + t] = a0, W3[4 * total + t] = a1, W3[5 * total + t] = a2;
      }
    }
  }
}

#define CH_NB 32
#define CH_LD (CH_NB + 4)
// ... 1087 lines not shown
```

henbun_amd/graph.py:

```python
from __future__ import annotations

import itertools
import math
from typing import Dict, List, Optional, Sequence, Tuple

import numpy as np

from ._lib import HipBackendError as _HipBackendError
from ._lib import constants as _constants

MATUTIL_BAND, MATUTIL_ADD_EYE, MATUTIL_PHI, MATUTIL_SYM, MATUTIL_SYMLOW = (
    _constants()["HB_MATUTIL_" + k] for k in ("BAND", "ADD_EYE", "PHI", "SYM", "SYMLOW"))

_uid = itertools.count()



class Node:
    __slots__ = ("op", "inputs", "attrs", "outputs", "id")

    def __init__(self, op, inputs, attrs, out_shapes):
        self.op = op
        self.inputs = tuple(inputs)
        self.attrs = attrs
# ... 808 lines not shown
    nd = len(vals[0].shape) + 1
    axis = axis % nd
    return concat([expand_dims(v, axis) for v in vals], axis)


def matmul(a, b, transpose_a=False, transpose_b=False, bias=None, act="none") -> Tensor:
    a, b = as_tensor(a), as_tensor(b)
    if len(a.shape) < 2 or len(b.shape) < 2:
        raise ValueError("matmul needs rank >= 2 operands")
    m, k = (a.shape[-1], a.shape[-2]) if transpose_a else (a.shape[-2], a.shape[-1])
    k2, n = (b.shape[-1], b.shape[-2]) if transpose_b else (b.shape[-2], b.shape[-1])
    if k != k2:
        raise ValueError("matmul inner dimensions differ: %s x %s" % (a.shape, b.shape))
    la, lb = a.shape[:-2], b.shape[:-2]
    if la and lb and la != lb:
        raise ValueError("matmul batch dimensions differ: %s vs %s" % (la, lb))
    lead = la if la else lb
    ins = (a, b) if bias is None else (a, b, as_tensor(bias))
    return make("matmul", ins, {"ta": bool(transpose_a), "tb": bool(transpose_b), "act": act},
                [tuple(lead) + (m, n)]).outputs[0]


def _matmul_emit(plan, node):
    H = plan.H
    if node.id in plan._phi_direct:
        return
    a, b = plan.buf(node.inputs[0]), plan.buf(node.inputs[1])
    bias = plan.buf(node.inputs[2]) if len(node.inputs) > 2 else None
    at = node.attrs
    y = node.outputs[0]
    g = getattr(plan, "_mm_head", {}).get(node.id)
    if g is not None:
        units = H.matmul_gauss_units(y.shape[0], node.inputs[0].shape[1], y.shape[1], plan.dtype)
        ok = (units > 0 and a.stride(1) == 1 and a.stride(0) % 4 == 0 and a.data_ptr() % 16 == 0 and b.stride(1) == 1
              and (bias is None or bias.numel() == y.shape[1]))
        if ok:
            def early(t):
                shp = t.shape
                while t.node.op == "reshape" and t not in plan._buf:
                    t = t.node.inputs[0]
                return plan.buf(t).view(shp)

            post = plan._gll_post.get(g.id)
            head = dict(y=early(g.inputs[0]), var=early(g.inputs[2]), scale=early(g.inputs[3]) if len(g.inputs) > 3 else None,
                        dmu=plan.out(g.outputs[1]), post=post[0] if post else 0.0, fbar=plan.out(post[1]) if post else None,
                        part=plan.scratch((3 * units,)), units=units)
            plan._gll_fused[g.id] = (head["part"], units)
            plan.pin_side_reads([g.inputs[0], g.inputs[2]] + list(g.inputs[3:4]))
            plan.steps.append(lambda: H.matmul_gauss(a, b, bias, head))
            return
        plan._gll_in_sgp.pop(g.id, None)
    cons = plan._consumers.get(y, [])
    epi = 0
    if (not at.get("actgrad") and len(cons) == 1 and cons[0].op == "matutil" and bias is None and at["act"] == "none" and y.shape[-1] == y.shape[-2]
            and y not in plan.outputs and y not in plan._bind):
        ma = cons[0].attrs
        epi = {MATUTIL_PHI: H.MM_PHI_OUT, MATUTIL_SYM: H.MM_SYM_OUT, MATUTIL_SYMLOW: H.MM_SYMLOW_OUT}.get(ma["mode"], 0)
        if ma["mode"] == MATUTIL_BAND and ma["lower"] < 0 and ma["upper"] == 0:
            epi = H.MM_TRIL_OUT
    if epi:
        out = plan.out(cons[0].outputs[0])
        plan._fused_matutil.add(cons[0].id)
    else:
        out = plan.out(y)
    csn = plan._colsum_of.get(node.id)
    if csn is not None and not epi:
        cout = plan.out(csn.outputs[0])
        plan.steps.append(lambda: H.matmul_colsum(a, b, out=out, colsum=cout))
        return
    if at.get("actgrad"):
        plan.steps.append(lambda: H.matmul(a, b, transA=at["ta"], transB=at["tb"], act=at["actgrad"], actgrad=bias, out=out))
        return
    ysh = y.shape
    kk = node.inputs[0].shape[-2] if at["ta"] else node.inputs[0].shape[-1]
    wgk_like = (plan.dtype == plan.torch.float32 and bias is None
                and H.matmul_wgk_shape(ysh[-2], ysh[-1], kk, int(np.prod(ysh[:-2])) if len(ysh) > 2 else 1))
    host = wgk_like and plan.attach_side(node)
    gg = cons[0] if (len(cons) == 1 and cons[0].op == "gram_grad") else None
    gp = "Gram VJP inside the product that computes Kbar (hb_matmul_gram_vjp)"
    if gg is not None and not epi and bias is None:
        from ._settings import settings as _st
        tX, tX2, tell, tg = gg.inputs
        B, BX, BX2, n, n2, d, sX, sX2, sEll, dl = _gram_layout(tX, tX2, tell)
        ok = (bool(getattr(_st.runtime, "gram_vjp_in_product", False)) and wgk_like and gg.attrs.get("sym") and tg is y
              and node.attrs.get("sym_result") and gg.attrs["kind"] == "rbf" and not (BX == 1 and B > 1) and y not in plan.outputs
              and y not in plan._bind and n == ysh[-1] and H.matmul_gram_vjp_ok(n, kk, B, d, plan.dtype))
        plan.note(gp, gg, ok, "" if ok else "needs the in-workgroup split-K form, the symmetric one-pass VJP of a UnitRBF Gram and d <= 4")
        if ok:
            X, ell = plan.buf(tX), plan.buf(tell)
            oX = plan.out(gg.outputs[0])
            lws = plan.scratch((max(B * n * d, 1),))
            part = plan.scratch((H.matmul_gram_vjp_ws_elems(B, n, d),))
            counters = plan.torch.zeros((B * (n // 32),), dtype=plan.torch.int32, device=plan.device)
            plan._gram_in_mm[gg.id] = (lws, (n if sEll != 0 else B * n), d, dl, (B if sEll != 0 else 1))
            plan.steps.append(lambda: H.matmul_gram_vjp(a, b, out, at["ta"], at["tb"], X, sX, ell, sEll, dl, d, oX, lws, part, counters))
            if host:
                plan.steps.append(lambda: H.side_flush())
            return
    plan.steps.append(lambda: H.matmul(a, b, transA=at["ta"], transB=at["tb"], bias=bias, act=at["act"], out=out,
                                       epilogue=epi))
    if host:
        plan.steps.append(lambda: H.side_flush())
    if csn is not None:
        cout, ra = plan.out(csn.outputs[0]), csn.attrs
        plan.steps.append(lambda: H.reduce_mid(b, ra["K1"], ra["R"], ra["K2"], op=H.RED_SUM, out=cout))


def _sum_lead(g, t):
    extra = len(g.shape) - len(t.shape)
    return reduce_sum(g, list(range(extra))) if extra > 0 else g


def _matmul_vjp(node, gs):
    g = gs[0]
    if g is None:
        return [None] * len(node.inputs)
    a, b = node.inputs[0], node.inputs[1]
    ta, tb, act = node.attrs["ta"], node.attrs["tb"], node.attrs["act"]
    y = node.outputs[0]
    if node.attrs.get("actgrad"):
        raise NotImplementedError("second derivatives through a fused activation-gradient GEMM are not supported")
    gn = g.node
    if (act != "none" and gn.op == "matmul" and len(gn.inputs) == 2 and gn.attrs["act"] == "none"
            and not gn.attrs.get("actgrad") and tuple(g.shape) == tuple(y.shape)):
        g = make("matmul", (gn.inputs[0], gn.inputs[1], y), {"ta": gn.attrs["ta"], "tb": gn.attrs["tb"], "act": "none",
                                                             "actgrad": act}, [tuple(g.shape)]).outputs[0]
    elif act == "sigmoid":
        g = binary("SIGMOID_GRAD", y, g)
    elif act == "tanh":
        g = binary("TANH_GRAD", y, g)
    elif act == "relu":
        g = binary("RELU_GRAD", y, g)
    if not ta:
        ga = matmul(g, b, transpose_b=not tb)
    else:
        ga = matmul(b, g, transpose_a=tb, transpose_b=True)
    if not tb:
        gb = matmul(a, g, transpose_a=not ta)
    else:
        gb = matmul(g, a, transpose_a=True, transpose_b=ta)
    res = [_sum_lead(ga, a), _sum_lead(gb, b)]
    if len(node.inputs) > 2:
        res.append(sum_to_shape(g, node.inputs[2].shape))
    return res


defop("matmul", _matmul_emit, _matmul_vjp)


def matutil(x, mode, lower=-1, upper=-1, alpha=0.0) -> Tensor:
    x = as_tensor(x)
    return make("matutil", (x,), {"mode": mode, "lower": int(lower), "upper": int(upper), "alpha": float(alpha)},
                [x.shape]).outputs[0]


def _known_lower(t) -> bool:
    n = t.node
    if n.op in ("cholesky", "trinv"):
        return True
    if n.op == "sgp_grad":
        return t.index == 0
    if n.op == "matutil":
        return n.attrs["mode"] == MATUTIL_PHI or (n.attrs["mode"] == MATUTIL_BAND and n.attrs["upper"] == 0)
    if n.op == "stop_gradient":
        return _known_lower(n.inputs[0])
    return False
# ... 392 lines not shown


def fullrank_sample_kl(mu, S, u=None, stream="global", packed=False) -> Tuple[Tensor, Tensor, Tensor]:
    mu, S = as_tensor(mu), as_tensor(S)
    size = mu.shape[-1]
    if packed:
        assert S.shape == mu.shape[:-1] + (size * (size + 1) // 2,)
    else:
        assert S.shape == mu.shape + (size,)
    ins = (mu, S) if u is None else (mu, S, as_tensor(u))
    n = make("fullrank_sample_kl", ins, {"stream": stream, "packed": bool(packed)}, [mu.shape, (1,), mu.shape],
             unique=u is None)
    return n.outputs[0], n.outputs[1], n.outputs[2]


def _fr_skl_emit(plan, node):
    H = plan.H
    mu, S = plan.buf(node.inputs[0]), plan.buf(node.inputs[1])
    u_in = plan.buf(node.inputs[2]) if len(node.inputs) > 2 else None
    outs = tuple(plan.out(t) for t in node.outputs)
    rng = None if u_in is not None else plan.rng(node.attrs["stream"])
    packed = bool(node.attrs.get("packed", False))
    plan.steps.append(lambda: H.fullrank_sample_kl_fwd(mu, S, u_in=u_in, rng=rng, out=outs, packed=packed))


def _fr_skl_vjp(node, gs):
    gx, gkl = gs[0], gs[1]
    if gx is None and gkl is None:
        return [None] * len(node.inputs)
    x, kl, u = node.outputs
    S = node.inputs[1]
    ins = [S, u, x]
    flags = {"has_x": gx is not None, "has_kl": gkl is not None, "packed": bool(node.attrs.get("packed", False))}
    if gx is not None:
        ins.append(gx)
    if gkl is not None:
        ins.append(gkl)
    n = make("fullrank_sample_kl_grad", tuple(ins), flags, [x.shape, S.shape])
    return [n.outputs[0], n.outputs[1]] + [None] * (len(node.inputs) - 2)


def _fr_skl_grad_emit(plan, node):
    H = plan.H
    bufs = [plan.buf(t) for t in node.inputs]
    S, u, x = bufs[:3]
    k = 3
    xbar = klbar = None
    if node.attrs["has_x"]:
        xbar = bufs[k]
        k += 1
    if node.attrs["has_kl"]:
        klbar = bufs[k]
    outs = tuple(plan.out(t) for t in node.outputs)
    packed = bool(node.attrs.get("packed", False))
    plan.steps.append(lambda: H.fullrank_sample_kl_bwd(S, u, x, xbar, klbar, out=outs, packed=packed))


defop("fullrank_sample_kl", _fr_skl_emit, _fr_skl_vjp)
defop("fullrank_sample_kl_grad", _fr_skl_grad_emit, None)


def vec_to_tri(v) -> Tensor:
    v = as_tensor(v)
    T = v.shape[-1]
    N = int((8 * T + 1) ** 0.5 / 2.0 - 0.5 + 1e-9)
    if N * (N + 1) // 2 != T:
        raise ValueError("vec_to_tri: %d is not a triangular number" % T)
    return make("vec_to_tri", (v,), {}, [v.shape[:-1] + (N, N)]).outputs[0]


def tri_to_vec(t) -> Tensor:
    t = as_tensor(t)
    N = t.shape[-1]
    assert t.shape[-2] == N
    return make("tri_to_vec", (t,), {}, [t.shape[:-2] + (N * (N + 1) // 2,)]).outputs[0]


defop("vec_to_tri", lambda plan, node: (lambda a, o: plan.steps.append(lambda: plan.H.vec_to_tri(a, out=o)))(
    plan.buf(node.inputs[0]), plan.out(node.outputs[0])), lambda node, gs: [None if gs[0] is None else tri_to_vec(gs[0])])
defop("tri_to_vec", lambda plan, node: (lambda a, o: plan.steps.append(lambda: plan.H.tri_to_vec(a, out=o)))(
    plan.buf(node.inputs[0]), plan.out(node.outputs[0])), lambda node, gs: [None if gs[0] is None else vec_to_tri(gs[0])])

KERN_KINDS = {"rbf": 0, "csym_rbf": 1, "sqdist": 2}


def gram(X, X2, ell, kind="rbf") -> Tensor:
    X, X2, ell = as_tensor(X), as_tensor(X2), as_tensor(ell)
    if X.shape[-1] != X2.shape[-1]:
        raise ValueError("gram: input dimensions differ")
    lead = X.shape[:-2] if len(X.shape) >= len(X2.shape) else X2.shape[:-2]
    if len(ell.shape) == 2 and ell.shape[0] > 1:
        if lead and int(np.prod(lead)) != ell.shape[0]:
            raise ValueError("gram: %d lengthscale sets for a batch of %s" % (ell.shape[0], lead))
        lead = lead or (ell.shape[0],)
    return make("gram", (X, X2, ell), {"kind": kind}, [tuple(lead) + (X.shape[-2], X2.shape[-2])]).outputs[0]


def _gram_layout(tX, tX2, tell):
    n, d = tX.shape[-2], tX.shape[-1]
    n2 = tX2.shape[-2]
    BX = int(np.prod(tX.shape[:-2])) if len(tX.shape) > 2 else 1
    BX2 = int(np.prod(tX2.shape[:-2])) if len(tX2.shape) > 2 else 1
    BE = tell.shape[0] if (len(tell.shape) == 2 and tell.shape[0] > 1) else 1
    B = max(BX, BX2, BE)
    sX = n * d if (BX == B and B > 1) else 0
    sX2 = n2 * d if (BX2 == B and B > 1) else 0
    dl = tell.size // BE
    sEll = dl if BE > 1 else 0
    return B, BX, BX2, n, n2, d, sX, sX2, sEll, dl


def _gram_emit(plan, node):
    H = plan.H
    X, X2, ell = (plan.buf(t) for t in node.inputs)
    k = KERN_KINDS[node.attrs["kind"]]
    y = node.outputs[0]
    cons = plan._consumers.get(y, [])
    if (len(cons) == 1 and cons[0].op == "matutil" and cons[0].attrs["mode"] == MATUTIL_ADD_EYE and y.shape[-1] == y.shape[-2]
            and y not in plan.outputs and y not in plan._bind):
        jit = cons[0].attrs["alpha"]
        kj = cons[0].outputs[0]
        cc = plan._consumers.get(kj, [])
        M = y.shape[-1]
        Bk = int(np.prod(y.shape[:-2])) if len(y.shape) > 2 else 1
        from ._settings import settings as _st

        if (bool(getattr(_st.runtime, "fold_gram", True)) and node.inputs[0] is node.inputs[1] and len(cc) == 1
                and cc[0].op == "cholesky" and kj not in plan.outputs
                and kj not in plan._bind and plan.dtype == plan.torch.float32 and k in (H.KERN_RBF, H.KERN_CSYM_RBF)
                and any(c.op == "trinv" for c in plan._consumers.get(cc[0].outputs[0], ()))
                and H.cholesky_persistent_shape(Bk, M, plan.dtype)):
            plan._fused_matutil.add(cons[0].id)
            plan._gram_for_chol[cc[0].id] = (X, ell, k, jit)
            plan.note("Gram folded into the persistent Cholesky (hb_gram_cholesky_inverse)", node, True)
            return
        plan.note("Gram folded into the persistent Cholesky (hb_gram_cholesky_inverse)", node, False,
                  "needs fp32, K(z, z) with one reader (a factor + inverse), an RBF-family kernel, M % 64 == 0 and "
                  "settings.runtime.fold_gram")
        out = plan.out(cons[0].outputs[0])
        plan._fused_matutil.add(cons[0].id)
        plan.steps.append(lambda: H.gram_fwd(X, X2, ell, kind=k, out=out, diag_add=jit))
        return
    out = plan.out(y)
    plan.steps.append(lambda: H.gram_fwd(X, X2, ell, kind=k, out=out))


def _gram_vjp(node, gs):
    g = gs[0]
    if g is None:
        return [None, None, None]
    X, X2, ell = node.inputs
    if X is X2:
        n = make("gram_grad", (X, X2, ell, g), {"kind": node.attrs["kind"], "sym": True}, [X.shape, ell.shape])
        return [n.outputs[0], None, n.outputs[1]]
    n = make("gram_grad", (X, X2, ell, g), {"kind": node.attrs["kind"], "sym": False}, [X.shape, X2.shape, ell.shape])
    return list(n.outputs)


def _gram_grad_emit(plan, node):
    H = plan.H
    fused = plan._gram_in_mm.get(node.id)
    if fused is not None:
        lws, rows, d_, dl_, groups = fused
        oL = plan.out(node.outputs[1])
        plan.out(node.outputs[0])
        fold = lambda: H.gram_ell_fold(lws, rows, d_, dl_, groups, oL)
        plan.steps.append(fold)
        plan.chain_kind[id(fold)] = "full"
        return
    tX, tX2, tell, tg = node.inputs
    X, X2, ell, g = (plan.buf(t) for t in node.inputs)
    k = KERN_KINDS[node.attrs["kind"]]
    B, BX, BX2, n, n2, d, sX, sX2, sEll, dl = _gram_layout(tX, tX2, tell)
    if node.attrs.get("sym"):
        oX, oL = [plan.out(t) for t in node.outputs]
        tmp = plan.scratch((B, n, d)) if (BX == 1 and B > 1) else None
        ws = plan.scratch((max(B * n * d, 1),))

        ksym = k | (H.KERN_KBAR_SYMMETRIC if tg.node.attrs.get("sym_result") else 0)

        def sym_step():
            dst = tmp if tmp is not None else oX
            H.gram_bwd_raw(ksym, X, sX, X2, sX2, ell, sEll, dl, g, dst, dst, oL, B, n, n2, d, ws)
            if tmp is not None:
                H.reduce_mid(tmp, 1, B, n * d, out=oX)

        plan.steps.append(sym_step)
        if tmp is None:
            plan.chain_kind[id(sym_step)] = "tail"
        return
    oX, oX2, oL = [plan.out(t) for t in node.outputs]
    tmpX = plan.scratch((B, n, d)) if (BX == 1 and B > 1) else None
    tmpX2 = plan.scratch((B, n2, d)) if (BX2 == 1 and B > 1) else None
    ws = plan.scratch((max(B * n * d, 1),))

    def step():
        H.gram_bwd_raw(k, X, sX, X2, sX2, ell, sEll, dl, g, tmpX if tmpX is not None else oX,
                       tmpX2 if tmpX2 is not None else oX2, oL, B, n, n2, d, ws)
        if tmpX is not None:
            H.reduce_mid(tmpX, 1, B, n * d, out=oX)
        if tmpX2 is not None:
            H.reduce_mid(tmpX2, 1, B, n2 * d, out=oX2)

    plan.steps.append(step)
    if tmpX is None and tmpX2 is None:
        plan.chain_kind[id(step)] = "tail"


defop("gram", _gram_emit, _gram_vjp)
defop("gram_grad", _gram_grad_emit, None)

SGP_MODES = {"neglected": 0, "diagonal": 1}


def sgp_samples(x, z, ell, L, u, mode="diagonal", eps=None) -> Tuple[Tensor, Tensor, Tensor, Tensor]:
    x, z, ell, L, u = (as_tensor(t) for t in (x, z, ell, L, u))
    W = stop_gradient(trinv(L))
    M, n, P = z.shape[-2], x.shape[-2], u.shape[-2]
    lead = z.shape[:-2]
    ins = [x, z, ell, L, W, u] + ([as_tensor(eps)] if eps is not None else [])
    nd = make("sgp", tuple(ins), {"mode": mode}, [lead + (P, n), lead + (M, n), lead + (n,), lead + (n,)],
              unique=(eps is None and mode == "diagonal"))
    return tuple(nd.outputs)


def _through_stop_gradient(t):
    while t.node.op == "stop_gradient":
        t = t.node.inputs[0]
    return t


def _sgp_emit(plan, node):
    H = plan.H
    x, z, ell, L, W, u = (plan.buf(t) for t in node.inputs[:6])
    eps_in = plan.buf(node.inputs[6]) if len(node.inputs) > 6 else None
    outs = tuple(plan.out(t) for t in node.outputs)
    mode = SGP_MODES[node.attrs["mode"]]
    rng = plan.rng("local") if (eps_in is None and mode == 1) else None
    wfrag, bf3 = plan._wfrag.get(_through_stop_gradient(node.inputs[4]), (None, False))
    bf3 = bf3 and node.inputs[0].shape[-1] <= 4 and node.inputs[5].shape[-2] <= 4
    prec = H.PREC_BF16X3 if bf3 else H.PREC_NATIVE
    zsh, xsh = node.inputs[1].shape, node.inputs[0].shape
    E, M, n, d, P = int(np.prod(zsh[:-2])) if len(zsh) > 2 else 1, zsh[-2], xsh[-2], xsh[-1], node.inputs[5].shape[-2]
# ... 684 lines not shown
        self._pending: List[tuple] = []
        if fuse and bool(getattr(_st.runtime, "head_in_contraction", True)):
            hoist_mb = self.side_jobs_enabled()

            def emitted_before(t, pos):
                while t.node.op == "reshape":
                    t = t.node.inputs[0]
                nd = t.node
                if nd.op == "leaf:minibatch" and hoist_mb:
                    return True
                cl = self._clusters.get(nd.id) or self._colclusters.get(nd.id)
                last = cl.nodes[-1] if (cl is not None and len(cl.nodes) >= 2) else nd
                return self._order_pos[last.id] < pos
            for n in order:
                if n.op != "gauss_ll" or len(n.inputs[1].shape) == 0:
                    continue
                ft = n.inputs[1]
                while ft.node.op == "reshape":
                    ft = ft.node.inputs[0]
                sg = ft.node
                hp = "likelihood head inside the forward contraction (hb_sgp_fwd_gauss)"
                if sg.op != "sgp" or ft is not sg.outputs[0] or sg.id in self._sgp_head or sg.inputs[5].shape[-2] != 1:
                    self.note(hp, n, False, "f is not the single latent function of an sgp draw" if sg.op != "sgp" or ft is not sg.outputs[0]
                              else ("the draw already carries a head" if sg.id in self._sgp_head else "more than one latent function (P > 1)"))
                    continue
                if n.inputs[0].size != ft.size:
                    self.note(hp, n, False, "y and f differ in size (a broadcast)")
                    continue
                pos = self._order_pos[sg.id]
                others = [n.inputs[0], n.inputs[2]] + list(n.inputs[3:4])
                if all(emitted_before(t, pos) for t in others):
                    self._sgp_head[sg.id] = n
                    self._gll_in_sgp[n.id] = sg
                    self.note(hp, n, True)
                else:
                    self.note(hp, n, False, "y / var / scale are produced after the draw is launched")
            self._mm_head: Dict[int, Node] = {}
            if bool(getattr(_st.runtime, "head_in_decoder", True)):
                hp = "likelihood head inside the layer's product (hb_matmul_gauss)"
                for n in order:
                    if n.op != "gauss_ll" or n.id in self._gll_in_sgp or len(n.inputs[1].shape) != 2:
                        continue
                    ft, single = n.inputs[1], True
                    while ft.node.op == "reshape":
                        single = single and len(consumers.get(ft, [])) == 1
                        ft = ft.node.inputs[0]
                    mm = ft.node
                    if mm.op != "matmul" or ft is not mm.outputs[0]:
                        continue
                    at = mm.attrs
                    why = None
                    if at["ta"] or at["tb"] or at.get("actgrad") or at["act"] != "none" or len(mm.inputs[0].shape) != 2 or len(mm.inputs[1].shape) != 2:
                        why = "the product is transposed, batched or carries an activation"
                    elif not single or len(consumers.get(ft, [])) != 1 or ft in self.outputs or ft in self._bind:
                        why = "f is read by something else as well"
                    elif n.inputs[0].shape != n.inputs[1].shape or mm.id in self._mm_head:
                        why = "y and f differ in shape"
                    elif not all(emitted_before(t, self._order_pos[mm.id]) for t in [n.inputs[0], n.inputs[2]] + list(n.inputs[3:4])):
                        why = "y / var / scale are produced after the product is launched"
                    elif hip_ops.matmul_gauss_units(ft.shape[0], mm.inputs[0].shape[1], ft.shape[1], dtype) == 0:
                        why = "shape outside the row-streaming form (fp32, n >= 2048, 32 < N <= 256, K = 16 / 32 / 64 / 128)"
                    if why is None:
                        self._mm_head[mm.id] = n
                        self._gll_in_sgp[n.id] = mm
                    self.note(hp, n, why is None, why or "")
        self._place: Dict[Tensor, object] = {}
        for n in order:
            if n.op != "concat":
                continue
            o, ax = n.outputs[0], n.attrs["axis"]
            if any(d != 1 for d in o.shape[:ax]):
                continue
            dst, off = None, 0
            for t in n.inputs:
                tgt = self._place_target(t)
                if (tgt is not None and tgt not in self._bind and tgt not in self._place and tgt not in self.outputs
                        and len(consumers.get(tgt, [])) == 1):
                    if dst is None:
                        dst = self.out(o).reshape(-1)
                    self._place[tgt] = dst[off:off + t.size].view(tgt.shape)
                off += t.size
        self._gram_for_chol: Dict[int, tuple] = {}
        self._gram_in_mm: Dict[int, tuple] = {}
        self._chol_rider: Dict[Tensor, dict] = {}
        self.step_riders: Dict[int, Node] = {}
        self._mlp2: Dict[int, dict] = {}
        self._colsum_of: Dict[int, Node] = {}
        self._fused_colsum = set()
        for n in order:
            if (n.op != "matmul" or not n.attrs["ta"] or n.attrs["tb"] or n.attrs.get("actgrad") or len(n.inputs) != 2
                    or n.attrs["act"] != "none" or len(n.inputs[0].shape) != 2 or len(n.inputs[1].shape) != 2):
                continue
            gmat = n.inputs[1]
            for r in consumers.get(gmat, []):
                ra = r.attrs if r.op == "reduce" else None
                if (ra is None or r.id in self._fused_colsum or ra["kind"] != "sum" or ra["K1"] != 1
                        or ra["R"] != gmat.shape[0] or ra["K2"] != gmat.shape[1]):
                    continue
                cl = self._clusters.get(r.id)
                if cl is not None and len(cl.nodes) > 1:
                    continue
                rout = r.outputs[0]
                if any(self._order_pos[c.id] < self._order_pos[n.id] for c in consumers.get(rout, [])):
                    continue
                self._colsum_of[n.id] = r
                self._fused_colsum.add(r.id)
                self.note("weight + bias gradient from one pass (hb_matmul_colsum)", n, True)
                break
        self._emitted: List[Node] = []
        self._side_cands: List[dict] = []
        hoisted = set()
        if self.side_jobs_enabled():
            for n in order:
                if n.op == "leaf:minibatch":
                    self._emit(n)
                    hoisted.add(n.id)
        for n in order:
            if n.id in hoisted:
                continue
            if n.id in self._absorbed:
                self._emitted.append(n)
                continue
            cc = self._colclusters.get(n.id)
            if cc is not None:
                if n is cc.nodes[-1]:
                    self._flush_pending([t for m in cc.nodes for t in m.inputs])
                    if self._emit_colcluster(cc):
                        self._emitted.extend(cc.nodes)
                continue
            c = self._clusters.get(n.id)
            if c is None or len(c.nodes) < 2:
                self._flush_pending(n.inputs)
                self._emit(n)
            elif n is c.nodes[-1]:
                self._flush_pending([t for m in c.nodes for t in m.inputs])
                self._emit_cluster(c)
                self._emitted.extend(c.nodes)
        self._flush_pending(None)
        for t, b in list(self._bind.items()) + self._extra_copies:
            got = self._buf.get(t)
            if got is not None and got.data_ptr() != b.data_ptr():
                src = got
                self.steps.append(lambda src=src, b=b: hip_ops.ewise("COPY", [src.reshape(b.shape)], out=b))

    def _prebind(self, t, b):
        n = t.node
        if n.op == "reshape":
            self._prebind(n.inputs[0], b.view(n.inputs[0].shape))
            return
        b = b.view(t.shape) if tuple(b.shape) != t.shape else b
        if t in self._bind:
            self._extra_copies.append((t, b))
        else:
            self._bind[t] = b

    def _flush_pending(self, reads):
        if not self._pending:
            return
        keep = []
        for step, label, node, writes in self._pending:
            if reads is None or any(t in writes for t in reads):
                self.steps.append(step)
                self.step_labels[id(step)] = label
                self.step_nodes[id(step)] = node
            else:
                keep.append((step, label, node, writes))
# ... 487 lines not shown
```

henbun_amd/hip_ops.py:

```python
from __future__ import annotations

import collections
import ctypes
from ctypes import c_double, c_int, c_long, c_void_p

import numpy as np
import torch

from . import _lib

_C = _lib.constants()


def _hb(*names):
    return [_C["HB_" + n] for n in names]


EW = {k[len("HB_EW_"):]: v for k, v in _C.items() if k.startswith("HB_EW_") and k != "HB_EW_PROG_SUM"}
RED_SUM, RED_MAX = _hb("RED_SUM", "RED_MAX")
KERN_RBF, KERN_CSYM_RBF, KERN_SQDIST = _hb("KERN_RBF", "KERN_CSYM_RBF", "KERN_SQDIST")
KERN_KBAR_SYMMETRIC = _C["HB_KERN_KBAR_SYMMETRIC"]
EW_PROG_SUM = _C["HB_EW_PROG_SUM"]
COLPROG_SUM, COLPROG_MAX = _hb("COLPROG_SUM", "COLPROG_MAX")
MM_LOWER_OUT, MM_TRIL_OUT, MM_PHI_OUT, MM_SYM_OUT = _hb("MM_LOWER_OUT", "MM_TRIL_OUT", "MM_PHI_OUT", "MM_SYM_OUT")
# ... 790 lines not shown
    B = L.numel() // max(M * M, 1)
    if out is None:
        out = _empty_like(L)
    ws = workspace(L.dtype, L.device, max(B * M * M, 1))
    _lib.lib().call("hb_trinv" + _suf(L), _p(L), _p(out), B, M, _p(ws), stream())
    return out


def _sgp_dims(x, z, u):
    E = z.shape[0] if z.dim() == 3 else 1
    M, d = z.shape[-2], z.shape[-1]
    n = x.shape[-2]
    P = u.shape[-2]
    sx = n * d if (x.dim() == 3 and x.shape[0] == E and E > 1) else 0
    return E, n, M, d, P, sx


def sgp_strip_path(E, n, M, d, P, prec=PREC_NATIVE):
    return bool(_lib.lib().raw("hb_sgp_strip_path")(E, n, M, d, P, int(prec)))


def sgp_frag_elems(E, n, M, prec=PREC_NATIVE):
    return int(_lib.lib().raw("hb_sgp_frag_elems")(int(E), int(n), int(M), int(prec)))


def _sgp_fwd_query(name, x, z, u, prec, has_wfrag, draw, rng):
    E, n, M, d, P, _ = _sgp_dims(x, z, u)
    if x.dtype != torch.float32:
        return 0
    return int(_lib.lib().raw(name)(E, n, M, d, P, int(prec), int(bool(has_wfrag)), int(bool(draw)), rng.nlanes if rng is not None else 0))


def sgp_head_units(x, z, u, prec, has_wfrag, draw, rng):
    return _sgp_fwd_query("hb_sgp_head_units", x, z, u, prec, has_wfrag, draw, rng)


def matmul_gram_vjp_ok(M, K, batch, d, dtype):
    if dtype != torch.float32:
        return False
    return bool(_lib.lib().raw("hb_matmul_gram_vjp_ok")(int(M), int(K), int(batch), int(d)))


def matmul_gram_vjp_ws_elems(batch, M, d):
    return int(_lib.lib().raw("hb_matmul_gram_vjp_ws_elems")(int(batch), int(M), int(d)))


def matmul_wgk_shape(M, N, K, batch):
    return bool(_lib.lib().raw("hb_matmul_wgk_shape")(int(M), int(N), int(K), int(batch)))


MatmulForm = collections.namedtuple("MatmulForm", "form S vec finish bfast colsum_fused")


def matmul_form(dtype, batch, M, N, K, lda=None, ldb=None, ldc=None, sA=None, sB=None, transA=False, transB=False, beta=0.0,
                flags=0, a_aligned=True, b_aligned=True, ws_elems=1 << 22, colsum=False):
    lda = (M if transA else K) if lda is None else lda
    ldb = (K if transB else N) if ldb is None else ldb
    ldc = N if ldc is None else ldc
    sA = (M * K if batch > 1 else 0) if sA is None else sA
    sB = (K * N if batch > 1 else 0) if sB is None else sB
    o = [ctypes.c_int(0) for _ in range(5)]
    form = _lib.lib().raw("hb_matmul_form")(_elem_bytes(dtype), int(batch), int(M), int(N), int(K), int(lda), int(ldb), int(ldc),
                                            int(sA), int(sB), int(bool(transA)), int(bool(transB)), float(beta), int(flags),
                                            int(bool(a_aligned)), int(bool(b_aligned)), int(ws_elems), int(bool(colsum)),
                                            *[ctypes.byref(v) for v in o])
    if form < 0:
        raise ValueError("matmul_form: an empty product, or arguments hb_matmul rejects")
    return MatmulForm(int(form), o[0].value, bool(o[1].value), bool(o[2].value), bool(o[3].value), bool(o[4].value))


def matmul_gram_vjp(a, b, out, transA, transB, X, sX, ell, sEll, dl, d, xbar, ell_partial, part, counters):
    M = out.shape[-1]
    batch = out.numel() // (M * M)
    K = a.shape[-2] if transA else a.shape[-1]
    sA = a.stride(0) if a.dim() == 3 and a.shape[0] > 1 else 0
    sB = b.stride(0) if b.dim() == 3 and b.shape[0] > 1 else 0
    _lib.lib().call("hb_matmul_gram_vjp_f32", _p(a), _p(b), _p(out), batch, M, K, a.stride(-2), b.stride(-2), out.stride(-2),
                    sA, sB, M * M, int(bool(transA)), int(bool(transB)), _p(X), int(sX), _p(ell), int(sEll), int(dl), int(d),
                    _p(xbar), _p(ell_partial), _p(part), _p(counters), stream())


def gram_ell_fold(partial, rows, d, dl, groups, ellbar):
    _lib.lib().call("hb_gram_ell_fold" + _suf(partial), _p(partial), int(rows), int(d), int(dl), int(groups), _p(ellbar), stream())


def matmul_gauss_units(n, K, N, dtype):
    if dtype != torch.float32:
        return 0
    return int(_lib.lib().raw("hb_matmul_gauss_units")(int(n), int(K), int(N)))


def matmul_gauss(x, w, bias, head):
    for t in (x, w):
        _chk(t)
    n, K = x.shape
    N = w.shape[1]
    _lib.lib().call("hb_matmul_gauss_f32", _p(x), x.stride(0), _p(w), w.stride(0), _p(bias), _p(head["y"]), _p(head.get("scale")),
                    _p(head["var"]), float(head.get("post") or 0.0), _p(head["dmu"]), _p(head.get("fbar")), _p(head["part"]),
                    int(head["units"]), int(n), int(K), int(N), stream())


def sgp_rider_supported(x, z, u, prec, has_wfrag, draw, rng):
    return bool(_sgp_fwd_query("hb_sgp_rider_supported", x, z, u, prec, has_wfrag, draw, rng))


def sgp_rider_begin():
    _lib.lib().call("hb_sgp_rider_begin")


def sgp_rider_flush():
    _lib.lib().call("hb_sgp_rider_flush", stream())


def sgp_rider_pending():
    return int(_lib.lib().raw("hb_sgp_rider_pending")())


def gauss_ll_fold(part, nb, ll, ds, dv):
    _lib.lib().call("hb_gauss_ll_fold" + _suf(part), _p(part), int(nb), _p(ll), _p(ds), _p(dv), stream())


def sgp_fwd(x, z, ell, W, u, eps_in=None, rng=None, mode=SGP_DIAGONAL, out=None, wfrag=None, prec=PREC_NATIVE,
            a_frag=None, skip_a=False, head=None):
    for t in (x, z, ell, W, u):
        _chk(t)
    E, n, M, d, P, sx = _sgp_dims(x, z, u)
    lead = (E,) if z.dim() == 3 else ()
    dev, dt = x.device, x.dtype
    if out is None:
        f = _empty(lead + (P, n), dtype=dt, device=dev)
        A = _empty(lead + (M, n), dtype=dt, device=dev)
        v = _empty(lead + (n,), dtype=dt, device=dev)
        eps = _empty(lead + (n,), dtype=dt, device=dev)
    else:
        f, A, v, eps = out
    dl = ell.numel() // E
    rp, rl = _rng_args(rng)
    ws = workspace(dt, dev, int(_lib.lib().raw("hb_sgp_ws_elems")(E, n, M, d, P)))
    if head is not None:
        _lib.lib().call("hb_sgp_fwd_gauss_f32", KERN_RBF, mode, _p(x), sx, _p(z), _p(ell), dl, _p(W), _p(wfrag), int(prec), _p(u),
                        _p(eps_in), rp, rl, _p(eps), None if (skip_a and a_frag is not None) else _p(A), _p(a_frag), _p(f), _p(v),
                        E, n, M, d, P, _p(ws), _p(head["y"]), _p(head.get("scale")), _p(head["var"]), float(head.get("post") or 0.0),
                        _p(head["dmu"]), _p(head.get("fbar")), _p(head["part"]), int(head["units"]), stream())
        return f, A, v, eps
    _lib.lib().call("hb_sgp_fwd" + _suf(x), KERN_RBF, mode, _p(x), sx, _p(z), _p(ell), dl, _p(W), _p(wfrag), int(prec), _p(u), _p(eps_in),
                    rp, rl, _p(eps), None if (skip_a and a_frag is not None) else _p(A), _p(a_frag), _p(f), _p(v), E, n,
                    M, d, P, _p(ws), stream())
    return f, A, v, eps


def sgp_A(x, z, ell, W, out=None, wfrag=None, prec=PREC_NATIVE):
    E = z.shape[0] if z.dim() == 3 else 1
    M, d = z.shape[-2], z.shape[-1]
    n = x.shape[-2]
    sx = n * d if (x.dim() == 3 and x.shape[0] == E and E > 1) else 0
    if out is None:
        out = _empty(((E,) if z.dim() == 3 else ()) + (M, n), dtype=x.dtype, device=x.device)
    _lib.lib().call("hb_sgp_A" + _suf(x), KERN_RBF, _p(x), sx, _p(z), _p(ell), ell.numel() // E, _p(W), _p(wfrag), int(prec),
                    _p(out), E, n, M, d, stream())
    return out


def sgp_predict_fused(dtype, E, n, M, d, P, s_kind, has_wfrag):
    return bool(_lib.lib().raw("hb_sgp_predict_fused")(int(E), int(n), int(M), int(d), int(P), int(s_kind), int(bool(has_wfrag)),
                                                       _elem_bytes(dtype)))

# ... 714 lines not shown
```

include/henbun_hip.h:

```cpp
#ifndef HENBUN_HIP_H
#define HENBUN_HIP_H

#include <stdint.h>

#ifdef __cplusplus
extern "C" {
#endif

#define HB_ABI_VERSION 2

int hb_version(void);
const char* hb_last_error_string(void);
int hb_debug_set(const char* key, long value);
int hb_debug_clear(void);
int hb_device_info(char* buf, int buflen, int* cu_count);

int hb_graph_begin_capture(void* stream);
int hb_graph_end_capture(void* stream, void** exec_out);
int hb_graph_launch(void* exec, void* stream);
int hb_graph_destroy(void* exec);

enum {
  HB_EW_NEG = 1, HB_EW_EXP, HB_EW_LOG, HB_EW_SQRT, HB_EW_SQUARE, HB_EW_ABS, HB_EW_SIGN,
  HB_EW_SIGMOID, HB_EW_RELU, HB_EW_SOFTPLUS, HB_EW_TANH, HB_EW_RECIP, HB_EW_RSQRT,
// ... 170 lines not shown
                  float* ws, long ws_elems, void* stream);
int hb_matmul_f64(const double* A, const double* B, double* C, long batch, long M, long N, long K,
                  long lda, long ldb, long ldc, long sA, long sB, long sC, int transA, int transB,
                  double alpha, double beta, const double* bias, long sBias, int act, int flags,
                  double* ws, long ws_elems, void* stream);

int hb_matmul_colsum_f32(const float* A, const float* B, float* C, float* colsum, long M, long N, long K, long lda, long ldb,
                         long ldc, float* ws, long ws_elems, void* stream);
int hb_matmul_colsum_f64(const double* A, const double* B, double* C, double* colsum, long M, long N, long K, long lda,
                         long ldb, long ldc, double* ws, long ws_elems, void* stream);

enum {
  HB_MM_FORM_TILE64 = 0,
  HB_MM_FORM_TILE128 = 1,
  HB_MM_FORM_WGK = 2,
  HB_MM_FORM_ROWS = 3,
  HB_MM_FORM_ROWSREG = 4
};
int hb_matmul_form(int elem_bytes, long batch, long M, long N, long K, long lda, long ldb, long ldc, long sA, long sB,
                   int transA, int transB, double beta, int flags, int a_aligned, int b_aligned, long ws_elems, int colsum,
                   int* S, int* vec, int* finish, int* bfast, int* colsum_fused);

int hb_mlp2_sample_supported(long n, long din, long hid, long nout, long rng_lanes, int has_u);
long hb_mlp2_sample_ws_elems(long n, long din, long hid);
int hb_mlp2_sample_fwd_f32(const float* y, const float* w0, const float* b0, const float* w1, const float* b1, int act,
                           const float* u_in, uint64_t* rng, long rng_lanes, float* x, float* kl, float* u_out, float* o,
                           long n, long din, long hid, float* ws, void* stream);
int hb_mlp2_sample_bwd_f32(const float* y, const float* w0, const float* b0, const float* w1, int act, const float* o,
                           const float* u, const float* x, const float* xbar, const float* klbar, float* dw0, float* db0,
                           float* dw1, float* db1, long n, long din, long hid, float* ws, void* stream);

int hb_cholesky_f32(const float* A, float* L, long B, long M, int* info, void* stream);
int hb_cholesky_f64(const double* A, double* L, long B, long M, int* info, void* stream);

long hb_cholesky_inverse_ws_elems(long B, long M, int elem_bytes);
long hb_cholesky_frag_elems(long B, long M, int bf16x3);
int hb_cholesky_persistent_shape(long B, long M, int elem_bytes);
int hb_gram_cholesky_inverse_f32(int kind, const float* X, long sX, const float* ell, long sEll, long dl, long d,
                                 double diag_add, float* L, float* W, long B, long M, int* info, float* ws,
                                 float* Wfrag, int frag_bf16x3, void* stream);
int hb_cholesky_inverse_f32(const float* A, float* L, float* W, long B, long M, int* info, float* ws,
                            float* Wfrag, int frag_bf16x3, void* stream);
int hb_cholesky_inverse_f64(const double* A, double* L, double* W, long B, long M, int* info,
                            double* ws, double* Wfrag, int frag_bf16x3, void* stream);
int hb_trinv_f32(const float* L, float* W, long B, long M, float* ws, void* stream);
int hb_trinv_f64(const double* L, double* W, long B, long M, double* ws, void* stream);

enum { HB_SGP_NEGLECTED = 0, HB_SGP_DIAGONAL = 1, HB_SGP_FULLRANK = 2  };
enum { HB_SGP_S_DIAG = 0, HB_SGP_S_TRIL = 1 };
enum { HB_PREC_NATIVE = 0, HB_PREC_BF16X3 = 1 };
long hb_sgp_ws_elems(long E, long n, long M, long d, long P);
int hb_sgp_strip_path(long E, long n, long M, long d, long P, int prec);
long hb_sgp_frag_elems(long E, long n, long M, int prec);
int hb_sgp_fwd_f32(int kind, int mode, const float* x, long sx, const float* z, const float* ell,
                   long dl, const float* W, const float* Wfrag, int prec, const float* u,
                   const float* eps_in, uint64_t* rng, long rng_lanes, float* eps_out, float* A,
                   float* A_frag, float* f, float* v, long E, long n, long M, long d, long P, float* ws,
                   void* stream);
int hb_sgp_fwd_f64(int kind, int mode, const double* x, long sx, const double* z, const double* ell,
                   long dl, const double* W, const double* Wfrag, int prec, const double* u,
                   const double* eps_in, uint64_t* rng, long rng_lanes, double* eps_out, double* A,
                   double* A_frag, double* f, double* v, long E, long n, long M, long d, long P,
                   double* ws, void* stream);
long hb_sgp_head_units(long E, long n, long M, long d, long P, int prec, int has_wfrag, int draw, long rng_lanes);
int hb_sgp_fwd_gauss_f32(int kind, int mode, const float* x, long sx, const float* z, const float* ell, long dl,
                         const float* W, const float* Wfrag, int prec, const float* u, const float* eps_in,
                         uint64_t* rng, long rng_lanes, float* eps_out, float* A, float* A_frag, float* f, float* v,
                         long E, long n, long M, long d, long P, float* ws, const float* y, const float* scale,
                         const float* var, double post, float* dmu, float* fbar, float* head_part, long units,
                         void* stream);
int hb_sgp_rider_supported(long E, long n, long M, long d, long P, int prec, int has_wfrag, int draw, long rng_lanes);
int hb_sgp_rider_begin(void);
int hb_sgp_rider_pending(void);
int hb_sgp_rider_flush(void* stream);
int hb_matmul_gram_vjp_ok(long M, long K, long batch, long d);
int hb_matmul_wgk_shape(long M, long N, long K, long batch);
long hb_matmul_gram_vjp_ws_elems(long batch, long M, long d);
int hb_matmul_gram_vjp_f32(const float* A, const float* B, float* C, long batch, long M, long K, long lda, long ldb,
                           long ldc, long sA, long sB, long sC, int transA, int transB, const float* X, long sX,
                           const float* ell, long sEll, long dl, long d, float* Xbar, float* ell_partial,
                           float* part, unsigned* counters, void* stream);
int hb_gram_ell_fold_f32(const float* partial, long rows, long d, long dl, long groups, float* ellbar, void* stream);
int hb_gram_ell_fold_f64(const double* partial, long rows, long d, long dl, long groups, double* ellbar, void* stream);
long hb_matmul_gauss_units(long n, long K, long N);
int hb_matmul_gauss_f32(const float* A, long lda, const float* B, long ldb, const float* bias, const float* y,
                        const float* scale, const float* var, double post, float* dmu, float* fbar, float* part,
                        long units, long n, long K, long N, void* stream);
int hb_gauss_ll_fold_f32(const float* partial, long nb, float* ll, float* dscale, float* dvar, void* stream);
int hb_gauss_ll_fold_f64(const double* partial, long nb, double* ll, double* dscale, double* dvar, void* stream);
int hb_sgp_A_f32(int kind, const float* x, long sx, const float* z, const float* ell, long dl,
                 const float* W, const float* Wfrag, int prec, float* A, long E, long n, long M, long d,
                 void* stream);
int hb_sgp_A_f64(int kind, const double* x, long sx, const double* z, const double* ell, long dl,
                 const double* W, const double* Wfrag, int prec, double* A, long E, long n, long M,
                 long d, void* stream);
long hb_sgp_predict_ws_elems(long E, long n, long M, long d, long P, int s_kind, int has_wfrag, int dtype_bytes);
int hb_sgp_predict_fused(long E, long n, long M, long d, long P, int s_kind, int has_wfrag, int dtype_bytes);
int hb_sgp_predict_f32(int kind, const float* x, long sx, const float* z, const float* ell, long dl, const float* W,
                       const float* Wfrag, const float* m, const float* s, int s_kind, int mode, double jitter, float* mean,
                       float* var, long E, long n, long M, long d, long P, float* ws, void* stream);
int hb_sgp_predict_f64(int kind, const double* x, long sx, const double* z, const double* ell, long dl, const double* W,
                       const double* Wfrag, const double* m, const double* s, int s_kind, int mode, double jitter,
                       double* mean, double* var, long E, long n, long M, long d, long P, double* ws, void* stream);
long hb_sgp_predict_cov_ws_elems(long E, long n, long M, long P, int s_kind, int dtype_bytes);
int hb_sgp_predict_cov_f32(int kind, const float* x, long sx, const float* z, const float* ell, long dl, const float* W,
                           const float* Wfrag, const float* s, int s_kind, int mode, double jitter, float* cov, long E, long n,
                           long M, long d, long P, float* ws, void* stream);
int hb_sgp_predict_cov_f64(int kind, const double* x, long sx, const double* z, const double* ell, long dl, const double* W,
                           const double* Wfrag, const double* s, int s_kind, int mode, double jitter, double* cov, long E,
                           long n, long M, long d, long P, double* ws, void* stream);
long hb_sgp_stats_ws_elems(long N, long M, long d, long P, int dtype_bytes);
int hb_sgp_stats_f32(int kind, const float* X, const float* Y, const float* z, const float* ell, long dl, const float* W,
                     const float* Wfrag, double* Phi, double* b, double* yy, double* a2sum, long N, long M, long d, long P,
                     float* ws, void* stream);
int hb_sgp_stats_f64(int kind, const double* X, const double* Y, const double* z, const double* ell, long dl, const double* W,
                     const double* Wfrag, double* Phi, double* b, double* yy, double* a2sum, long N, long M, long d, long P,
                     double* ws, void* stream);
long hb_sgp_wstats_ws_elems(long N, long M, long d, int dtype_bytes);
int hb_sgp_wstats_f32(int kind, const float* X, const float* w, const float* r, const float* z, const float* ell, long dl,
                      const float* W, const float* Wfrag, double* Phi, double* b, double* tr, long N, long M, long d, float* ws,
                      void* stream);
int hb_sgp_wstats_f64(int kind, const double* X, const double* w, const double* r, const double* z, const double* ell, long dl,
                      const double* W, const double* Wfrag, double* Phi, double* b, double* tr, long N, long M, long d,
                      double* ws, void* stream);
enum { HB_LIK_GAUSSIAN = 0, HB_LIK_BERNOULLI = 1, HB_LIK_POISSON = 2 };
long hb_lik_sites_ws_elems(long N);
int hb_lik_sites_f32(int lik, const float* y, const float* mean, const float* var, double mscale, double vscale, double param,
                     float* lam, float* beta, double* ell_sum, long N, double* ws, void* stream);
int hb_lik_sites_f64(int lik, const double* y, const double* mean, const double* var, double mscale, double vscale,
                     double param, double* lam, double* beta, double* ell_sum, long N, double* ws, void* stream);
int hb_lik_predict_f32(int lik, const float* mean, const float* var, double param, float* ymean, float* yvar, long N,
                       void* stream);
int hb_lik_predict_f64(int lik, const double* mean, const double* var, double param, double* ymean, double* yvar, long N,
                       void* stream);
int hb_sgp_pathwise_f32(int kind, const float* x, const float* omega, const float* z, const float* ell, long dl,
                        const float* coef, double scale, float* out, long n, long L, long M, long d, long S, void* stream);
int hb_sgp_pathwise_f64(int kind, const double* x, const double* omega, const double* z, const double* ell, long dl,
                        const double* coef, double scale, double* out, long n, long L, long M, long d, long S, void* stream);
int hb_sgp_pathwise_grad_f32(int kind, const float* x, const float* omega, const float* z, const float* ell, long dl,
                             const float* coef, double scale, float* out, float* grad, long n, long L, long M, long d, long S,
                             void* stream);
int hb_sgp_pathwise_grad_f64(int kind, const double* x, const double* omega, const double* z, const double* ell, long dl,
                             const double* coef, double scale, double* out, double* grad, long n, long L, long M, long d, long S,
                             void* stream);
long hb_sgp_pathwise_argmax_ws_elems(long n, long S);
int hb_sgp_pathwise_argmax_f32(int kind, const float* x, const float* omega, const float* z, const float* ell, long dl,
                               const float* coef, double scale, int largest, float* best, long* idx, long n, long L, long M,
                               long d, long S, float* ws, void* stream);
int hb_sgp_pathwise_argmax_f64(int kind, const double* x, const double* omega, const double* z, const double* ell, long dl,
                               const double* coef, double scale, int largest, double* best, long* idx, long n, long L, long M,
                               long d, long S, double* ws, void* stream);
enum { HB_PWACQ_EI = 0, HB_PWACQ_PI = 1 };
long hb_sgp_pathwise_acq_ws_elems(long n, long S);
int hb_sgp_pathwise_acq_f32(int kind, const float* x, const float* omega, const float* z, const float* ell, long dl,
                            const float* coef, double scale, int acq, int largest, const float* incumbent, float* value,
                            float* best, long* idx, long n, long L, long M, long d, long S, double* ws, void* stream);
int hb_sgp_pathwise_acq_f64(int kind, const double* x, const double* omega, const double* z, const double* ell, long dl,
                            const double* coef, double scale, int acq, int largest, const double* incumbent, double* value,
                            double* best, long* idx, long n, long L, long M, long d, long S, double* ws, void* stream);
enum { HB_ACQ_EI = 0, HB_ACQ_PI = 1, HB_ACQ_UCB = 2 };
long hb_sgp_predict_grad_ws_elems(long n, long M, long d, int s_kind, int has_wfrag, int dtype_bytes);
int hb_sgp_predict_grad_f32(int kind, const float* x, const float* z, const float* ell, long dl, const float* W,
                            const float* Wfrag, const float* m, const float* s, int s_kind, int mode, double jitter,
                            float* mean, float* var, float* dmean, float* dvar, long n, long M, long d, float* ws,
                            void* stream);
int hb_sgp_predict_grad_f64(int kind, const double* x, const double* z, const double* ell, long dl, const double* W,
// ... 124 lines not shown
```

Measured before the change: 43.52 million samples/s.

## Fold RBF Gram VJP into Kbar product epilogue with tile partials and chain fold

Adds a tiles variant of the Kbar-producing matmul. Its epilogue computes the RBF Gram VJP contributions for each 32x32 tile, warp-reduces them, and writes per-tile partials without storing Kbar. A new chain job then folds these partials into Xbar and the lengthscale gradient inside the serial chain kernel. This removes the materialised MxM Kbar and the separate Gram backward pass, at the cost of more epilogue work and an added partial buffer. The path is enabled by default when the shape and lengthscale conditions hold.

```diff
diff --git a/henbun_amd/csrc/chain.cuh b/henbun_amd/csrc/chain.cuh
--- a/henbun_amd/csrc/chain.cuh
+++ b/henbun_amd/csrc/chain.cuh
@@ -3,7 +3,7 @@
 #include "common.cuh"
 #include "ew_prog.cuh"
 
-enum { HB_CHAIN_PROG = 1, HB_CHAIN_ADAM = 2, HB_CHAIN_GLL = 3, HB_CHAIN_SGP_FINISH = 4, HB_CHAIN_GRAM_ELL = 5, HB_CHAIN_GLL_FOLD = 6 };
+enum { HB_CHAIN_PROG = 1, HB_CHAIN_ADAM = 2, HB_CHAIN_GLL = 3, HB_CHAIN_SGP_FINISH = 4, HB_CHAIN_GRAM_ELL = 5, HB_CHAIN_GLL_FOLD = 6, HB_CHAIN_GRAM_TILES = 7 };
 #define HB_CHAIN_MAX_JOBS 6
 #define HB_CHAIN_PROG_MAX_N 4096
 #define HB_CHAIN_FINISH_MAX_N 512
@@ -11,6 +11,7 @@
 #define HB_CHAIN_ADAM_MAX_N 4096
 #define HB_CHAIN_ELL_MAX_N 16384
 #define HB_CHAIN_GLL_FOLD_MAX_N 4096
+#define HB_CHAIN_TILES_MAX_N 16384
 
 enum { HB_CHAIN_READ = 1, HB_CHAIN_WRITE = 2, HB_CHAIN_RW = 3 };
 
diff --git a/henbun_amd/csrc/chain_bodies.cuh b/henbun_amd/csrc/chain_bodies.cuh
--- a/henbun_amd/csrc/chain_bodies.cuh
+++ b/henbun_amd/csrc/chain_bodies.cuh
@@ -369,6 +369,72 @@
   hb_gram_ell_body<T, 1>(h, partial, rows, d, dl, c, ellbar, smem, mir);
 }
 
+#define HB_GRAM_TILES_MAXD 4
+__device__ __forceinline__ long hb_gram_tiles_addr(long o, long tiles_n, long d) {
+  const unsigned w = 64u * (unsigned)d, g = (unsigned)o / w;
+  return (long)(g * (unsigned)tiles_n * w + ((unsigned)o - g * w));
+}
+template <typename T, int S, int TN>
+__device__ __forceinline__ void hb_gram_tiles_load(const T* __restrict__ part, long outs, long d, T (&h)[S * TN > 0 ? S * TN : 1]) {
+#pragma unroll
+  for (int s = 0; s < S; ++s) {
+    const long o = (long)threadIdx.x + (long)s * blockDim.x, oc = o < outs ? o : outs - 1;
+    const T* p = part + hb_gram_tiles_addr(oc, TN, d);
+#pragma unroll
+    for (int t = 0; t < TN; ++t) h[s * TN + t] = p[(long)t * 64 * d];
+  }
+}
+template <typename T, int S, int TN, typename F>
+__device__ __forceinline__ void hb_gram_tiles_body(const T (&h)[S * TN > 0 ? S * TN : 1], const T* __restrict__ part, long outs, long tiles_n, long d,
+                                                   long dl, T* __restrict__ Xbar, T* __restrict__ ellbar, T* smem, F on_xbar,
+                                                   T* mir = nullptr) {
+  T lp[HB_GRAM_TILES_MAXD];
+#pragma unroll
+  for (int k = 0; k < HB_GRAM_TILES_MAXD; ++k) lp[k] = T(0);
+  auto put = [&](long o, T v) {
+    const long row = (long)((unsigned)o / (2u * (unsigned)d)), q = o - row * 2 * d;
+    if (q < d) {
+      Xbar[row * d + q] = v;
+      on_xbar(Xbar + row * d + q, v);
+    } else {
+      const long c = dl == 1 ? 0 : q - d;
+#pragma unroll
+      for (int k = 0; k < HB_GRAM_TILES_MAXD; ++k)
+        if (c == k) lp[k] += v;
+    }
+  };
+#pragma unroll
+  for (int s = 0; s < S; ++s) {
+    const long o = (long)threadIdx.x + (long)s * blockDim.x;
+    T acc = T(0);
+#pragma unroll
+    for (int t = 0; t < TN; ++t) acc += h[s * TN + t];
+    if (o < outs) put(o, acc);
+  }
+  for (long o = (long)threadIdx.x + (long)S * blockDim.x; o < outs; o += blockDim.x) {
+    const T* p = part + hb_gram_tiles_addr(o, tiles_n, d);
+    T acc = T(0);
+    for (long t = 0; t < tiles_n; ++t) acc += p[t * 64 * d];
+    put(o, acc);
+  }
+#pragma unroll
+  for (int k = 0; k < HB_GRAM_TILES_MAXD; ++k) {
+    if (k < dl) {
+      const T e = block_sum(lp[k], smem);
+      if (threadIdx.x == 0) {
+        ellbar[k] = e;
+        if (mir && k == 0) mir[0] = e;
+      }
+    }
+  }
+}
+template <typename T, typename F>
+__device__ __forceinline__ void hb_gram_tiles_body(const T* __restrict__ part, long outs, long tiles_n, long d, long dl,
+                                                   T* __restrict__ Xbar, T* __restrict__ ellbar, T* smem, F on_xbar) {
+  const T h[1] = {T(0)};
+  hb_gram_tiles_body<T, 0, 1, F>(h, part, outs, tiles_n, d, dl, Xbar, ellbar, smem, on_xbar);
+}
+
 template <typename T, int D>
 __device__ __forceinline__ void hb_chain_win_load(const T* base, long n, T (&h)[D]) {
 #pragma unroll
diff --git a/henbun_amd/csrc/gram.hip b/henbun_amd/csrc/gram.hip
--- a/henbun_amd/csrc/gram.hip
+++ b/henbun_amd/csrc/gram.hip
@@ -201,6 +201,31 @@
   return gram_ell_fold<double>(partial, rows, d, dl, groups, ellbar, (hipStream_t)stream);
 }
 
+__global__ void __launch_bounds__(1024) gram_tiles_fold_kernel(const float* __restrict__ part, long outs, long tiles_n, long d, long dl,
+                                                               float* __restrict__ Xbar, float* __restrict__ ellbar) {
+  __shared__ float smem[16];
+  hb_gram_tiles_body<float>(part, outs, tiles_n, d, dl, Xbar, ellbar, smem, HbNoMirror());
+}
+extern "C" int hb_gram_tiles_fold_f32(const float* part, long batch, long M, long d, long dl, float* Xbar, float* ellbar, void* stream) {
+  HB_REQUIRE(part && Xbar && ellbar, "hb_gram_tiles_fold: NULL pointer");
+  HB_REQUIRE(batch >= 1 && M >= 32 && M % 32 == 0 && d >= 1 && d <= HB_GRAM_TILES_MAXD && (dl == 1 || dl == d), "hb_gram_tiles_fold: bad arguments");
+  const long tiles = M / 32, elems = batch * tiles * tiles * 64 * d;
+  HB_REQUIRE(elems <= HB_CHAIN_TILES_MAX_N, "hb_gram_tiles_fold: %ld partials, more than one workgroup folds (%d)", elems, HB_CHAIN_TILES_MAX_N);
+  if (hb_chain_recording()) {
+    HbChainJob j;
+    j.kind = HB_CHAIN_GRAM_TILES;
+    j.is64 = 0;
+    j.p[0] = part, j.p[1] = Xbar, j.p[2] = ellbar;
+    j.l[0] = batch * M * 2 * d, j.l[1] = tiles, j.l[2] = d, j.l[3] = dl;
+    j.span(0, elems * (long)sizeof(float), HB_CHAIN_READ);
+    j.span(1, batch * M * d * (long)sizeof(float), HB_CHAIN_WRITE), j.span(2, dl * (long)sizeof(float), HB_CHAIN_WRITE);
+    return hb_chain_push(j, (hipStream_t)stream);
+  }
+  hipLaunchKernelGGL(gram_tiles_fold_kernel, dim3(1), dim3(1024), 0, (hipStream_t)stream, part, batch * M * 2 * d, tiles, d, dl, Xbar, ellbar);
+  HB_LAUNCH_CHECK();
+  return 0;
+}
+
 extern "C" int hb_gram_bwd_f32(int kind, const float* X, long sX, const float* X2, long sX2, const float* ell,
                                long sEll, long dl, const float* Kbar, float* Xbar, float* X2bar, float* ellbar,
                                long B, long n, long n2, long d, float* ws, void* stream) {
diff --git a/henbun_amd/csrc/jit.hip b/henbun_amd/csrc/jit.hip
--- a/henbun_amd/csrc/jit.hip
+++ b/henbun_amd/csrc/jit.hip
@@ -474,6 +474,7 @@
     case HB_CHAIN_GLL_FOLD: *p = 4, *l = 1, *d = 0; break;
     case HB_CHAIN_SGP_FINISH: *p = 6, *l = 6, *d = 0; break;
     case HB_CHAIN_GRAM_ELL: *p = 2, *l = 4, *d = 0; break;
+    case HB_CHAIN_GRAM_TILES: *p = 3, *l = 4, *d = 0; break;
     default: *p = 20, *l = 8, *d = 8; break;
   }
 }
@@ -532,6 +533,11 @@
                  "      hb_gram_ell_body<T>((const T*)A.p[%d] + grp * A.l[%d] * A.l[%d], A.l[%d], A.l[%d], A.l[%d], c, "
                  "(T*)A.p[%d] + grp * A.l[%d], smem);\n",
               l0 + 3, l0 + 2, p0, l0, l0 + 1, l0, l0 + 1, l0 + 2, p0 + 1, l0 + 2);
+    } else if (j.kind == HB_CHAIN_GRAM_TILES) {
+      const int p0 = P(j.p[0]); P(j.p[1]); P(j.p[2]);
+      const int l0 = L(j.l[0]); L(j.l[1]); L(j.l[2]); L(j.l[3]);
+      appendf(s, "  hb_gram_tiles_body<T>((const T*)A.p[%d], A.l[%d], A.l[%d], A.l[%d], A.l[%d], (T*)A.p[%d], (T*)A.p[%d], smem, HbNoMirror());\n",
+              p0, l0, l0 + 1, l0 + 2, l0 + 3, p0 + 1, p0 + 2);
     } else {
       HB_REQUIRE(false, "hb_chain: unknown job kind %d", j.kind);
     }
@@ -605,6 +611,7 @@
       case HB_CHAIN_GLL: return k >= 5 && k <= 7 ? 1 : 0;
       case HB_CHAIN_GLL_FOLD: return k >= 1 && k <= 3 ? 1 : 0;
       case HB_CHAIN_GRAM_ELL: return k == 1 && J.ext[1] == (long)esz ? 1 : 0;
+      case HB_CHAIN_GRAM_TILES: return k == 1 ? 2 : (k == 2 && J.ext[2] == (long)esz ? 1 : 0);
       default: return 0;
     }
   }
@@ -726,6 +733,9 @@
     } else if (j.kind == HB_CHAIN_GRAM_ELL) {
       c.part_ext = plan.external(q, 0);
       c.depth = (int)(((j.l[2] == 1 ? j.l[0] * j.l[1] : j.l[0]) + 1023) / 1024);
+    } else if (j.kind == HB_CHAIN_GRAM_TILES) {
+      c.part_ext = plan.external(q, 0);
+      c.depth = (int)((j.l[0] + 1023) / 1024);
     }
     if (c.depth < 1) c.depth = 1;
   }
@@ -749,6 +759,8 @@
         if (c.part_ext && !fits(3 * c.depth)) c.part_ext = false;
       } else if (j.kind == HB_CHAIN_GRAM_ELL) {
         if (c.part_ext && !fits(c.depth)) c.part_ext = false;
+      } else if (j.kind == HB_CHAIN_GRAM_TILES) {
+        if (c.part_ext && !fits(c.depth * (int)j.l[1])) c.part_ext = false;
       } else if (j.kind == HB_CHAIN_PROG) {
         for (int k = 0; k < j.prog.nin; ++k)
           if (c.in[k].kind == CH_EXT && !fits(1)) c.in[k].kind = CH_PLAIN;
@@ -884,6 +896,19 @@
                  "(T*)A.p[%d] + grp * A.l[%d], smem, %s);\n",
               l0 + 3, c.part_ext ? "(grp == 0 ? 1L : 0L)" : "0L", l0 + 2, p0, l0, l0 + 1, l0, l0 + 1, l0 + 2, p0 + 1, l0 + 2,
               c.part_ext ? "(T*)nullptr" : mir.c_str());
+    } else if (j.kind == HB_CHAIN_GRAM_TILES) {
+      const int p0 = P(j.p[0]); P(j.p[1]); P(j.p[2]);
+      const int l0 = L(j.l[0]); L(j.l[1]); L(j.l[2]); L(j.l[3]);
+      std::string fn = "HbNoMirror()";
+      const std::string mt = plan.mirror_text(q, 1);
+      if (!mt.empty()) fn = "[&](const T* hp, T hv) { " + hook_text(mt, "hp", "hv") + "}";
+      const int S = c.part_ext ? c.depth : 0, TN = c.part_ext ? (int)j.l[1] : 1;
+      if (c.part_ext)
+        appendf(top, "  T h%dp[%d]; hb_gram_tiles_load<T, %d, %d>((const T*)A.p[%d], A.l[%d], A.l[%d], h%dp);\n", q, S * TN, S, TN, p0, l0, l0 + 2, q);
+      else
+        appendf(s, "  const T h%dp[1] = {T(0)};\n", q);
+      appendf(s, "  hb_gram_tiles_body<T, %d, %d>(h%dp, (const T*)A.p[%d], A.l[%d], A.l[%d], A.l[%d], A.l[%d], (T*)A.p[%d], (T*)A.p[%d], smem, %s, %s);\n",
+              S, TN, q, p0, l0, l0 + 1, l0 + 2, l0 + 3, p0 + 1, p0 + 2, fn.c_str(), plan.mir_arg(q, 2).c_str());
     } else {
       HB_REQUIRE(false, "hb_chain: unknown job kind %d", j.kind);
     }
diff --git a/henbun_amd/csrc/linalg.hip b/henbun_amd/csrc/linalg.hip
--- a/henbun_amd/csrc/linalg.hip
+++ b/henbun_amd/csrc/linalg.hip
@@ -2,6 +2,7 @@
 #include "sgp_strip.cuh"
 #include "side_jobs.cuh"
 #include "gemm_tile.cuh"
+#include "chain.cuh"
 #include "../../include/henbun_hip.h"
 
 template <typename T>
@@ -279,7 +280,48 @@
   unsigned* counters = nullptr;
 };
 #define HB_MMG_MAXD 4
-template <bool TA, bool TB, bool SYM>
+template <int D>
+__device__ __forceinline__ void wgk_tiles_vjp(const float (&gval)[4], const float (&pxi)[4][HB_MMG_MAXD], const float (&pxj)[HB_MMG_MAXD],
+                                              const float (&pel)[HB_MMG_MAXD], float* __restrict__ pt, int tid) {
+  float il[D], v[4][2 * D];
+#pragma unroll
+  for (int k = 0; k < D; ++k) il[k] = 1.f / pel[k];
+#pragma unroll
+  for (int e = 0; e < 4; ++e) {
+    float dm[D], r2 = 0.f;
+#pragma unroll
+    for (int k = 0; k < D; ++k) {
+      dm[k] = pxi[e][k] * il[k] - pxj[k] * il[k];
+      r2 += dm[k] * dm[k];
+    }
+    const float km = hb_exp(-0.5f * r2), kb = gval[e];
+    const float em = kb * km, gm = (kb + kb) * km;
+#pragma unroll
+    for (int k = 0; k < D; ++k) {
+      v[e][k] = (-dm[k] * gm) * il[k];
+      v[e][D + k] = (dm[k] * dm[k] * em) * il[k];
+    }
+  }
+#pragma unroll
+  for (int off = 16; off > 0; off >>= 1) {
+    float t[4][2 * D];
+#pragma unroll
+    for (int e = 0; e < 4; ++e)
+#pragma unroll
+      for (int q = 0; q < 2 * D; ++q) t[e][q] = __shfl_xor(v[e][q], off, 32);
+#pragma unroll
+    for (int e = 0; e < 4; ++e)
+#pragma unroll
+      for (int q = 0; q < 2 * D; ++q) v[e][q] += t[e][q];
+  }
+  if ((tid & 31) == 0) {
+#pragma unroll
+    for (int e = 0; e < 4; ++e)
+#pragma unroll
+      for (int q = 0; q < 2 * D; ++q) pt[((tid >> 5) + 8 * e) * 2 * D + q] = v[e][q];
+  }
+}
+template <bool TA, bool TB, bool SYM, bool TILES = false>
 __global__ void __launch_bounds__(256) matmul_wgk_kernel(MmArgs<float> a, int nown, HbSideJobs side, MmGramVjp gv) {
   if ((int)blockIdx.x >= nown) {
     if (blockIdx.y == 0) hb_side_run(side, (int)blockIdx.x - nown);
@@ -363,6 +405,20 @@
       }
     }
   };
+  float pxj[HB_MMG_MAXD], pxi[4][HB_MMG_MAXD], pel[HB_MMG_MAXD];
+  if (TILES) {
+    const int d = (int)gv.d;
+    const float* Xb = gv.X + b * gv.sX;
+    const float* eb = gv.ell + b * gv.sEll;
+#pragma unroll
+    for (int k = 0; k < HB_MMG_MAXD; ++k) {
+      const int kc = k < d ? k : 0;
+      pel[k] = eb[gv.dl == 1 ? 0 : kc];
+      pxj[k] = Xb[(long)(col0 + (tid & 31)) * d + kc];
+#pragma unroll
+      for (int e = 0; e < 4; ++e) pxi[e][k] = Xb[(long)(row0 + (tid >> 5) + 8 * e) * d + kc];
+    }
+  }
   {
     Frag fa, fb;
     load(fa, 0);
@@ -408,9 +464,19 @@
     if (a.beta != 0.f) v += a.beta * Cb[gr * a.ldc + gcn];
     if ((a.flags & (HB_MM_TRIL_OUT | HB_MM_PHI_OUT)) && gcn > gr) v = 0.f;
     if ((a.flags & HB_MM_PHI_OUT) && gcn == gr) v *= 0.5f;
-    Cb[gr * a.ldc + gcn] = v;
-  }
-  if (!SYM && gv.X) {
+    if (!TILES || a.C != nullptr) Cb[gr * a.ldc + gcn] = v;
+  }
+  if (!SYM && TILES) {
+    const int d = (int)gv.d;
+    float* pt = gv.part + ((((long)b * (M / 32) + ti) * tiles_n + tj) * 32) * 2 * d;
+    switch (d) {
+      case 1: wgk_tiles_vjp<1>(gval, pxi, pxj, pel, pt, tid); break;
+      case 2: wgk_tiles_vjp<2>(gval, pxi, pxj, pel, pt, tid); break;
+      case 3: wgk_tiles_vjp<3>(gval, pxi, pxj, pel, pt, tid); break;
+      default: wgk_tiles_vjp<4>(gval, pxi, pxj, pel, pt, tid); break;
+    }
+  }
+  if (!SYM && !TILES && gv.X) {
     const int d = (int)gv.d, c = tid & 31;
     const float* Xb = gv.X + b * gv.sX;
     const float* eb = gv.ell + b * gv.sEll;
@@ -504,10 +570,10 @@
 }
 template <typename T>
 static int matmul_wgk_launch(const MmArgs<T>&, int, int, hipStream_t) { return -1; }
-int matmul_wgk_launch_g(const MmArgs<float>& a, int transA, int transB, hipStream_t stream, const MmGramVjp& gv);
+int matmul_wgk_launch_g(const MmArgs<float>& a, int transA, int transB, hipStream_t stream, const MmGramVjp& gv, bool tiles = false);
 template <>
 int matmul_wgk_launch<float>(const MmArgs<float>& a, int transA, int transB, hipStream_t stream) { return matmul_wgk_launch_g(a, transA, transB, stream, MmGramVjp()); }
-int matmul_wgk_launch_g(const MmArgs<float>& a, int transA, int transB, hipStream_t stream, const MmGramVjp& gv) {
+int matmul_wgk_launch_g(const MmArgs<float>& a, int transA, int transB, hipStream_t stream, const MmGramVjp& gv, bool tiles) {
   const bool sym = (a.flags & HB_MM_SYM_OUT) != 0;
   const long nt = a.M / 32;
   const int nown = (int)(sym ? nt * (nt + 1) / 2 : (a.M / 32) * (a.N / 32));
@@ -517,6 +583,8 @@
   do {                                                                                                     \
     if (sym)                                                                                               \
       hipLaunchKernelGGL((matmul_wgk_kernel<TA_, TB_, true>), grid, dim3(256), 0, stream, a, nown, sj, gv);    \
+    else if (tiles)                                                                                        \
+      hipLaunchKernelGGL((matmul_wgk_kernel<TA_, TB_, false, true>), grid, dim3(256), 0, stream, a, nown, sj, gv); \
     else                                                                                                   \
       hipLaunchKernelGGL((matmul_wgk_kernel<TA_, TB_, false>), grid, dim3(256), 0, stream, a, nown, sj, gv);   \
   } while (0)
@@ -1216,6 +1284,32 @@
   gv.X = X, gv.sX = sX, gv.ell = ell, gv.sEll = sEll, gv.dl = dl, gv.d = d;
   gv.Xbar = Xbar, gv.ell_partial = ell_partial, gv.part = part, gv.counters = counters;
   return matmul_wgk_launch_g(a, transA, transB, (hipStream_t)stream, gv);
+}
+
+extern "C" int hb_matmul_gram_vjp_tiles_ok(long M, long K, long batch, long d) {
+  if (hb_debug_get("gram_vjp_tiles", 1) == 0 || !hb_matmul_gram_vjp_ok(M, K, batch, d)) return 0;
+  return hb_matmul_gram_vjp_ws_elems(batch, M, d) <= HB_CHAIN_TILES_MAX_N ? 1 : 0;
+}
+extern "C" int hb_matmul_gram_vjp_tiles_f32(const float* A, const float* B, float* C, long batch, long M, long K, long lda, long ldb,
+                                            long ldc, long sA, long sB, long sC, int transA, int transB, const float* X, long sX,
+                                            const float* ell, long sEll, long dl, long d, float* part, void* stream) {
+  HB_REQUIRE(A && B && X && ell && part, "hb_matmul_gram_vjp_tiles: NULL pointer");
+  HB_REQUIRE(hb_matmul_gram_vjp_tiles_ok(M, K, batch, d), "hb_matmul_gram_vjp_tiles: shape outside the tiles form (hb_matmul_gram_vjp_tiles_ok)");
+  HB_REQUIRE(dl == 1 || dl == d, "hb_matmul_gram_vjp_tiles: lengthscales must have 1 or d entries");
+  HB_REQUIRE(sX == 0 || sX == M * d, "hb_matmul_gram_vjp_tiles: point batch stride must be 0 or M * d");
+  HB_REQUIRE(sEll == 0 || sEll == dl, "hb_matmul_gram_vjp_tiles: lengthscale batch stride must be 0 or dl");
+  if (C == nullptr) ldc = M, sC = 0;
+  const bool aligned = ((uintptr_t)A % 16 == 0) && ((uintptr_t)B % 16 == 0) && ((uintptr_t)C % 16 == 0) && lda % 4 == 0 && ldb % 4 == 0 && ldc % 4 == 0;
+  HB_REQUIRE(aligned, "hb_matmul_gram_vjp_tiles: operands must be 16-byte aligned with leading dimensions %% 4 == 0");
+  HB_REQUIRE(lda >= (transA ? M : K) && ldb >= (transB ? K : M) && ldc >= M, "hb_matmul_gram_vjp_tiles: leading dimension too small");
+  MmArgs<float> a = {};
+  a.A = A, a.B = B, a.C = C;
+  a.M = M, a.N = M, a.K = K, a.lda = lda, a.ldb = ldb, a.ldc = ldc, a.sA = sA, a.sB = sB, a.sC = sC, a.batch = batch;
+  a.alpha = 1.f, a.beta = 0.f, a.act = HB_ACT_NONE, a.flags = 0;
+  MmGramVjp gv;
+  gv.X = X, gv.sX = sX, gv.ell = ell, gv.sEll = sEll, gv.dl = dl, gv.d = d;
+  gv.part = part;
+  return matmul_wgk_launch_g(a, transA, transB, (hipStream_t)stream, gv, true);
 }
 
 static inline bool matmul_gauss_shape(long n, long K, long N, int& G, int& KC) {
diff --git a/henbun_amd/graph.py b/henbun_amd/graph.py
--- a/henbun_amd/graph.py
+++ b/henbun_amd/graph.py
@@ -914,6 +914,20 @@
         from ._settings import settings as _st
         tX, tX2, tell, tg = gg.inputs
         B, BX, BX2, n, n2, d, sX, sX2, sEll, dl = _gram_layout(tX, tX2, tell)
+        pair = (wgk_like and gg.attrs.get("sym") and tg is y and node.attrs.get("sym_result") and gg.attrs["kind"] == "rbf"
+                and not (BX == 1 and B > 1) and y not in plan.outputs and y not in plan._bind and n == ysh[-1])
+        tiles = bool(pair and sEll == 0 and not getattr(_st.runtime, "gram_vjp_in_product", False)
+                     and H.matmul_gram_vjp_tiles_ok(n, kk, B, d, plan.dtype))
+        plan.note(GRAM_TILES, gg, tiles, "" if tiles else "needs the pairing of the in-product Gram VJP, lengthscales shared by the batch, at most "
+                  "16384 tile partials (hb_matmul_gram_vjp_tiles_ok) and hb_debug_set gram_vjp_tiles 1")
+        if tiles:
+            X, ell = plan.buf(tX), plan.buf(tell)
+            part = plan.scratch((H.matmul_gram_vjp_ws_elems(B, n, d),))
+            plan._gram_tiles[gg.id] = (part, B, n, d, dl)
+            plan.steps.append(lambda: H.matmul_gram_vjp_tiles(a, b, None, at["ta"], at["tb"], X, sX, ell, sEll, dl, d, part))
+            if host:
+                plan.steps.append(lambda: H.side_flush())
+            return
         ok = (bool(getattr(_st.runtime, "gram_vjp_in_product", False)) and wgk_like and gg.attrs.get("sym") and tg is y
               and node.attrs.get("sym_result") and gg.attrs["kind"] == "rbf" and not (BX == 1 and B > 1) and y not in plan.outputs
               and y not in plan._bind and n == ysh[-1] and H.matmul_gram_vjp_ok(n, kk, B, d, plan.dtype))
@@ -1472,6 +1486,7 @@
     plan.buf(node.inputs[0]), plan.out(node.outputs[0])), lambda node, gs: [None if gs[0] is None else vec_to_tri(gs[0])])
 
 KERN_KINDS = {"rbf": 0, "csym_rbf": 1, "sqdist": 2}
+GRAM_TILES = "Gram VJP's tile partials from the product that computes Kbar, folded by the serial chain (hb_matmul_gram_vjp_tiles)"
 
 
 def gram(X, X2, ell, kind="rbf") -> Tensor:
@@ -1549,6 +1564,14 @@
 
 def _gram_grad_emit(plan, node):
     H = plan.H
+    tiles = plan._gram_tiles.get(node.id)
+    if tiles is not None:
+        part, B_, n_, d_, dl_ = tiles
+        oX, oL = plan.out(node.outputs[0]), plan.out(node.outputs[1])
+        fold = lambda: H.gram_tiles_fold(part, B_, n_, d_, dl_, oX, oL)
+        plan.steps.append(fold)
+        plan.chain_kind[id(fold)] = "full"
+        return
     fused = plan._gram_in_mm.get(node.id)
     if fused is not None:
         lws, rows, d_, dl_, groups = fused
@@ -2399,6 +2422,7 @@
                 off += t.size
         self._gram_for_chol: Dict[int, tuple] = {}
         self._gram_in_mm: Dict[int, tuple] = {}
+        self._gram_tiles: Dict[int, tuple] = {}
         self._chol_rider: Dict[Tensor, dict] = {}
         self.step_riders: Dict[int, Node] = {}
         self._mlp2: Dict[int, dict] = {}
diff --git a/henbun_amd/hip_ops.py b/henbun_amd/hip_ops.py
--- a/henbun_amd/hip_ops.py
+++ b/henbun_amd/hip_ops.py
@@ -896,6 +896,27 @@
 
 def gram_ell_fold(partial, rows, d, dl, groups, ellbar):
     _lib.lib().call("hb_gram_ell_fold" + _suf(partial), _p(partial), int(rows), int(d), int(dl), int(groups), _p(ellbar), stream())
+
+
+def matmul_gram_vjp_tiles_ok(M, K, batch, d, dtype):
+    if dtype != torch.float32:
+        return False
+    return bool(_lib.lib().raw("hb_matmul_gram_vjp_tiles_ok")(int(M), int(K), int(batch), int(d)))
+
+
+def matmul_gram_vjp_tiles(a, b, out, transA, transB, X, sX, ell, sEll, dl, d, part):
+    M = a.shape[-1] if transA else a.shape[-2]
+    K = a.shape[-2] if transA else a.shape[-1]
+    batch = a.numel() // (M * K) if a.dim() == 3 else (b.numel() // (M * K) if b.dim() == 3 else 1)
+    sA = a.stride(0) if a.dim() == 3 and a.shape[0] > 1 else 0
+    sB = b.stride(0) if b.dim() == 3 and b.shape[0] > 1 else 0
+    _lib.lib().call("hb_matmul_gram_vjp_tiles_f32", _p(a), _p(b), _p(out) if out is not None else None, batch, M, K, a.stride(-2),
+                    b.stride(-2), out.stride(-2) if out is not None else M, sA, sB, M * M, int(bool(transA)), int(bool(transB)),
+                    _p(X), int(sX), _p(ell), int(sEll), int(dl), int(d), _p(part), stream())
+
+
+def gram_tiles_fold(part, batch, M, d, dl, xbar, ellbar):
+    _lib.lib().call("hb_gram_tiles_fold_f32", _p(part), int(batch), int(M), int(d), int(dl), _p(xbar), _p(ellbar), stream())
 
 
 def matmul_gauss_units(n, K, N, dtype):
diff --git a/include/henbun_hip.h b/include/henbun_hip.h
--- a/include/henbun_hip.h
+++ b/include/henbun_hip.h
@@ -276,6 +276,11 @@
                            float* part, unsigned* counters, void* stream);
 int hb_gram_ell_fold_f32(const float* partial, long rows, long d, long dl, long groups, float* ellbar, void* stream);
 int hb_gram_ell_fold_f64(const double* partial, long rows, long d, long dl, long groups, double* ellbar, void* stream);
+int hb_matmul_gram_vjp_tiles_ok(long M, long K, long batch, long d);
+int hb_matmul_gram_vjp_tiles_f32(const float* A, const float* B, float* C, long batch, long M, long K, long lda, long ldb,
+                                 long ldc, long sA, long sB, long sC, int transA, int transB, const float* X, long sX,
+                                 const float* ell, long sEll, long dl, long d, float* part, void* stream);
+int hb_gram_tiles_fold_f32(const float* part, long batch, long M, long d, long dl, float* Xbar, float* ellbar, void* stream);
 long hb_matmul_gauss_units(long n, long K, long N);
 int hb_matmul_gauss_f32(const float* A, long lda, const float* B, long ldb, const float* bias, const float* y,
                         const float* scale, const float* var, double post, float* dmu, float* fbar, float* part,
```

After: 44.33 million samples/s, median of 6. 1.02x the previous value.
